# JuliaNeuralGraphics/GaussianSplatting.jl

Hardware: AMD Instinct MI355X
Metric: fwd+bwd Mpixels/s @1920x1080, 1M Gaussians SH=3 (higher is better)
Workload: dtype f32

## Files before the change

### gaussiansplatting.jl_amd/_lib.py

```python
from __future__ import annotations

import ctypes as C
import os
import subprocess

_HERE = os.path.dirname(os.path.abspath(__file__))
LIB_PATH = os.environ.get("GSR_HIP_LIB", os.path.join(_HERE, "libgsr_hip.so"))
HEADER_PATH = os.path.join(os.path.dirname(_HERE), "include", "gsr.h")

GSR_OK, GSR_E_INVALID_ARG, GSR_E_OOM, GSR_E_HIP, GSR_E_STATE = 0, -1, -2, -3, -4
DEFAULT = 0
SSIM_FAST, SSIM_EXACT = 1, 2
PREPROCESS_DIRECT, PREPROCESS_AGGREGATING = 1, 2
TUNER_OFF, TUNER_ON = 1, 2
GRAD_FP32_REFERENCE, GRAD_ACCURATE = 1, 2
MODES = {"rgb": 3, "rgbd": 5, "rgbdn": 8}
FORWARD_ONLY = 1
FLAG_REFERENCE_TILE_LISTS = 2
FLAG_ANTIALIASED = 4
ABI_VERSION = 6

(BUF_RADII, BUF_GRAD_MEANS2D, BUF_N_CONTRIB, BUF_FINAL_T, BUF_TILE_RANGES, BUF_VALUES_SORTED, BUF_GEOM, BUF_NORMALS,
 BUF_GRAD_ROWS, BUF_INSTANCE_AUX, BUF_COMPENSATIONS) = range(11)


class GsrError(RuntimeError):
    def __init__(self, code, msg):
        super().__init__(f"gsr error {code}: {msg}")
        self.code = code


class Config(C.Structure):
    _fields_ = [("width", C.c_int32), ("height", C.c_int32), ("mode", C.c_int32), ("near_plane", C.c_float),
                ("far_plane", C.c_float), ("radius_clip", C.c_int32), ("blur_eps", C.c_float), ("flags", C.c_uint32),
                ("bins_budget_bytes", C.c_uint64), ("ssim_precision", C.c_int32), ("preprocess_form", C.c_int32),
                ("form_tuner", C.c_int32), ("grad_precision", C.c_int32)]


class Inputs(C.Structure):
    _fields_ = [("n", C.c_int32), ("n_coeffs", C.c_int32), ("sh_degree", C.c_int32), ("means", C.c_void_p),
                ("shs", C.c_void_p), ("opacities", C.c_void_p), ("scales", C.c_void_p), ("rotations", C.c_void_p),
                ("background", C.c_float * 3)]


class CameraS(C.Structure):
    _fields_ = [("R", C.c_float * 9), ("t", C.c_float * 3), ("focal", C.c_float * 2), ("principal", C.c_float * 2),
                ("camera_center", C.c_float * 3), ("R_dev", C.c_void_p), ("t_dev", C.c_void_p)]


class Aux(C.Structure):
    _fields_ = [("covisibilities", C.c_void_p), ("uncertainties", C.c_void_p), ("radii", C.c_void_p),
                ("flags", C.c_uint32), ("reserved", C.c_uint32)]


class Stats(C.Structure):
    _fields_ = [("n_rendered", C.c_int64), ("n_visible", C.c_int32), ("max_tile_instances", C.c_int32),
                ("generation", C.c_uint64), ("bins_bytes", C.c_int64), ("compact_binning", C.c_int32), ("preprocess_form", C.c_int32),
                ("bins_regrowths", C.c_uint32), ("compact_fallbacks", C.c_uint32), ("tuner_rearms", C.c_uint32),
                ("scratch_regrowths", C.c_uint32), ("fused_relaunches", C.c_uint32), ("held_views", C.c_uint32),
                ("bin_capacity", C.c_uint32), ("tuner_form", C.c_int32), ("tuner_ms", C.c_float * 2),
                ("tier_tiles", C.c_uint32 * 3), ("reserved", C.c_uint32)]

    HISTORY = ("bins_regrowths", "compact_fallbacks", "tuner_rearms", "scratch_regrowths", "fused_relaunches", "held_views")

    def history(self) -> dict:
        return {k: int(getattr(self, k)) for k in self.HISTORY}


class Grads(C.Structure):
    _fields_ = [("vmeans", C.c_void_p), ("vshs", C.c_void_p), ("vopacities", C.c_void_p), ("vscales", C.c_void_p),
                ("vrotations", C.c_void_p), ("vR", C.c_void_p), ("vt", C.c_void_p), ("vcolors", C.c_void_p),
                ("vmeans2d", C.c_void_p), ("forward_generation", C.c_uint64), ("flags", C.c_uint32), ("reserved", C.c_uint32)]


GRADS_COLOR_COTANGENT = 0x1
ADAM_MAX_GROUPS = 8


class AdamGroup(C.Structure):
    _fields_ = [("theta", C.c_void_p), ("grad", C.c_void_p), ("mu", C.c_void_p), ("nu", C.c_void_p),
                ("count", C.c_int64), ("lr", C.c_float), ("current_step", C.c_uint32)]


class TailGrads(C.Structure):
    _fields_ = [("vmeans", C.c_void_p), ("vshs", C.c_void_p), ("vopacities", C.c_void_p), ("vscales", C.c_void_p),
                ("vrotations", C.c_void_p)]


class TailState(C.Structure):
    _fields_ = [("theta", C.c_void_p * 6), ("mu", C.c_void_p * 6), ("nu", C.c_void_p * 6), ("lr", C.c_float * 6),
                ("current_step", C.c_uint32 * 6), ("beta1", C.c_float), ("beta2", C.c_float), ("eps", C.c_float),
                ("scale_dims", C.c_int32), ("shs", C.c_void_p), ("opacities_act", C.c_void_p),
                ("scales_act", C.c_void_p), ("vmeans2d", C.c_void_p), ("forward_generation", C.c_uint64),
                ("flags", C.c_uint32), ("reserved", C.c_uint32)]


class ComposeGroup(C.Structure):
    _fields_ = [("src", C.c_void_p), ("dst", C.c_void_p), ("row_words", C.c_int32), ("new_zero", C.c_int32)]


class DepthAnchorS(C.Structure):
    _fields_ = [("a", C.c_float), ("b", C.c_float), ("floor", C.c_float), ("disparity", C.c_float), ("p_far", C.c_float)]


COMPOSE_MAX_GROUPS = 24
FILTER3D_CAMERA_FLOATS = 22
DENSIFY_CLONE, DENSIFY_SPLIT, DENSIFY_PRUNE = 0, 1, 2


class GatherGroup(C.Structure):
    _fields_ = [("src", C.c_void_p), ("dst", C.c_void_p), ("row_words", C.c_int32)]


class FormTuner(C.Structure):
    _fields_ = [("phase", C.c_int32), ("form", C.c_int32), ("n_ref", C.c_int32), ("age", C.c_uint32), ("ms", C.c_float * 2)]


class PolicyConfig(C.Structure):
    _fields_ = [("grid_x", C.c_int32), ("grid_y", C.c_int32), ("bins_budget_bytes", C.c_uint64), ("preprocess_form", C.c_int32),
                ("form_tuner", C.c_int32), ("beside_max_tiles", C.c_uint32), ("bwd_split_max_tiles", C.c_uint32),
                ("agg_max_bands", C.c_int32), ("reserved", C.c_int32)]


class PolicyState(C.Structure):
    _fields_ = [("bin_cap", C.c_uint32), ("compact_sticky", C.c_uint32), ("last_n", C.c_int32), ("last_max_tile", C.c_uint32),
                ("last_n_rendered", C.c_int64), ("tier_n", C.c_uint32 * 3), ("bin_cap_view", C.c_uint32), ("views", C.c_uint64),
                ("tuner", FormTuner), ("bins_regrowths", C.c_uint32), ("compact_fallbacks", C.c_uint32),
                ("compact_views", C.c_uint32), ("overflow_views", C.c_uint32), ("tuner_rearms", C.c_uint32),
                ("fused_relaunches", C.c_uint32), ("held_views", C.c_uint32), ("reserved", C.c_uint32)]


class ViewPlan(C.Structure):
    _fields_ = [("bin_cap_view", C.c_uint32), ("form_request", C.c_int32), ("form", C.c_int32), ("timed_slot", C.c_int32),
                ("skewed", C.c_int32), ("hold_fused", C.c_int32), ("tuner_decided", C.c_int32), ("spec_mid4", C.c_uint32),
                ("spec_mid8", C.c_uint32), ("reserved", C.c_int32)]


class ViewOutcome(C.Structure):
    _fields_ = [("binning", C.c_int32), ("fused_done", C.c_int32), ("long_tiles", C.c_int32), ("beside", C.c_int32),
                ("launch_fused_now", C.c_int32), ("reserved", C.c_int32), ("sorted_mid4", C.c_uint32), ("sorted_mid8", C.c_uint32),
                ("bin_cap_next", C.c_uint32), ("bins_regrown", C.c_uint32)]


class BwdSplit(C.Structure):
    _fields_ = [("n_big", C.c_uint32), ("n_mid8", C.c_uint32), ("n_mid4", C.c_uint32), ("split_len", C.c_uint32)]


POLICY_EXPORTS = ["gsr_policy_config_init", "gsr_policy_state_init", "gsr_policy_agg_plan", "gsr_policy_preprocess_form",
                  "gsr_policy_form_is_open", "gsr_policy_begin_view", "gsr_policy_end_view", "gsr_policy_bwd_split"]


def bind_policy(lib):
    P = C.POINTER
    lib.gsr_policy_config_init.argtypes = [P(PolicyConfig), C.c_int32, C.c_int32, C.c_uint64, C.c_int32]
    lib.gsr_policy_config_init.restype = None
    lib.gsr_policy_state_init.argtypes = [P(PolicyState)]
    lib.gsr_policy_state_init.restype = None
    lib.gsr_policy_agg_plan.argtypes = [C.c_int32, C.c_int32, C.c_uint32, P(C.c_int32), P(C.c_int32), P(C.c_size_t), P(C.c_int32)]
    lib.gsr_policy_agg_plan.restype = None
    lib.gsr_policy_preprocess_form.argtypes = [P(PolicyConfig), C.c_int32, C.c_int32, C.c_uint32, C.c_int32]
    lib.gsr_policy_preprocess_form.restype = C.c_int32
    lib.gsr_policy_form_is_open.argtypes = [P(PolicyConfig), C.c_int32, C.c_uint32]
    lib.gsr_policy_form_is_open.restype = C.c_int32
    lib.gsr_policy_begin_view.argtypes = [P(PolicyConfig), P(PolicyState), C.c_int32, P(C.c_float), P(ViewPlan)]
    lib.gsr_policy_begin_view.restype = None
    lib.gsr_policy_end_view.argtypes = [P(PolicyConfig), P(PolicyState), P(ViewPlan), C.c_int64, C.c_uint32, C.c_uint32, C.c_uint32,
                                        C.c_uint32, C.c_uint64, C.c_int32, P(ViewOutcome)]
    lib.gsr_policy_end_view.restype = None
    lib.gsr_policy_bwd_split.argtypes = [P(PolicyConfig), C.c_uint32, C.c_uint32, C.c_uint32, P(BwdSplit)]
    lib.gsr_policy_bwd_split.restype = None
    lib.gsr_bins_capacity_after.argtypes = [C.c_int64, C.c_int32, C.c_int32, C.c_int32, C.c_uint64, C.c_uint32]
    lib.gsr_bins_capacity_after.restype = C.c_uint32
    return lib


EXPORTS = ["gsr_create", "gsr_destroy", "gsr_release_scene_buffers", "gsr_memory_usage", "gsr_debug_check_guards", "gsr_reserve", "gsr_drop_forward", "gsr_bins_capacity_after", "gsr_forward",
           "gsr_backward", "gsr_host_wait_policy", "gsr_buffer", "gsr_copy_buffer", "gsr_ssim_forward", "gsr_ssim_backward", "gsr_loss_l1_ssim",
           "gsr_ssim_precision", "gsr_get_ssim_precision", "gsr_preprocess_form", "gsr_get_preprocess_form",
           "gsr_allreduce_grads", "gsr_last_error_string", "gsr_version", "gsr_abi_version", "gsr_check_abi", "gsr_profile_enable",
           "gsr_profile_stage_count", "gsr_profile_stages", "gsr_profile_stage_name", "gsr_profile_read", "gsr_profile_read_intervals", "gsr_update_stats",
           "gsr_prologue_forward", "gsr_prologue_backward", "gsr_adam_step", "gsr_stream_triad",
           "gsr_mask_findall_scratch_bytes", "gsr_mask_findall", "gsr_gather_rows", "gsr_sh_grad_from_views", "gsr_sh_grad_from_views_tail", "gsr_trainer_tail_step",
           "gsr_backward_trainer_tail",
           "gsr_densify_grad_mean", "gsr_densify_mask", "gsr_compose_rows", "gsr_split_transform", "gsr_reset_opacity", "gsr_morton_codes",
           "gsr_knn_scratch_bytes", "gsr_knn_scales",
           "gsr_filter3d_scratch_bytes", "gsr_filter3d_compute", "gsr_filter3d_apply", "gsr_filter3d_apply_backward",
           "gsr_tsdf_integrate", "gsr_mesh_scratch_bytes", "gsr_mesh_count", "gsr_mesh_emit",
           "gsr_ply_pack_rows", "gsr_ply_unpack_rows", "gsr_count_nonfinite",
           "gsr_bilateral_scratch_bytes", "gsr_bilateral_tv_scratch_bytes", "gsr_bilateral_slice_forward",
           "gsr_bilateral_slice_backward", "gsr_bilateral_tv", "gsr_bilateral_adam_tail",
           "gsr_normal_loss_scratch_bytes", "gsr_normal_loss_forward", "gsr_normal_loss_backward",
           "gsr_flatten_loss_scratch_bytes", "gsr_flatten_loss",
           "gsr_depth_loss_scratch_bytes", "gsr_depth_target", "gsr_depth_loss_forward", "gsr_depth_loss_backward",
           "gsr_sky_scratch_bytes", "gsr_sky_composite_forward", "gsr_sky_composite_backward",
           "gsr_eval_scratch_bytes", "gsr_eval_metrics", "gsr_frame_rgb8",
           "gsr_frames_scratch_bytes", "gsr_depth_scale", "gsr_frame_depth16", "gsr_frame_normal8", "gsr_pick_point",
           "gsr_mcmc_weights", "gsr_mcmc_sample_scratch_bytes", "gsr_mcmc_sample", "gsr_mcmc_split_sampled",
           "gsr_mcmc_relocation_params", "gsr_mcmc_relocate_rows", "gsr_mcmc_inject_noise",
           "gsr_mcmc_regularization_scratch_bytes", "gsr_mcmc_regularization"] + POLICY_EXPORTS

_lib = None


def build(verbose: bool = False) -> str:
    cmd = ["make", "-C", os.path.join(_HERE, "csrc"), "-j4"]
    r = subprocess.run(cmd, capture_output=True, text=True)
    if verbose or r.returncode != 0:
        print(r.stdout[-4000:], r.stderr[-4000:])
    if r.returncode != 0:
        raise RuntimeError("building libgsr_hip.so failed")
    return LIB_PATH


def build_tools(verbose: bool = False) -> bool:
    r = subprocess.run(["make", "-C", os.path.join(_HERE, "csrc"), "tools"], capture_output=True, text=True)
    if verbose or r.returncode != 0:
        print(r.stdout[-2000:], r.stderr[-2000:])
    return r.returncode == 0


def load():
    global _lib
    if _lib is not None:
        return _lib
    if not os.path.exists(LIB_PATH):
        raise RuntimeError(f"{LIB_PATH} is missing: run __graft_entry__.build() (there is no CPU fallback)")
    import torch
    lib = C.CDLL(LIB_PATH)
    vp, i32, f32 = C.c_void_p, C.c_int, C.c_float
    lib.gsr_create.argtypes = [C.POINTER(Config), C.POINTER(vp)]
    lib.gsr_destroy.argtypes = [vp]
    lib.gsr_release_scene_buffers.argtypes = [vp]
    lib.gsr_memory_usage.argtypes = [vp]
    lib.gsr_memory_usage.restype = C.c_int64
    lib.gsr_debug_check_guards.argtypes = [vp]
    lib.gsr_reserve.argtypes = [vp, C.c_int64, C.c_int64]
    lib.gsr_drop_forward.argtypes = [vp]
    bind_policy(lib)
    lib.gsr_forward.argtypes = [vp, C.POINTER(Inputs), C.POINTER(CameraS), vp, C.POINTER(Aux), vp, C.POINTER(Stats)]
    lib.gsr_backward.argtypes = [vp, C.POINTER(Inputs), C.POINTER(CameraS), vp, C.POINTER(Grads), vp]
    lib.gsr_host_wait_policy.argtypes = [i32, i32, i32]
    lib.gsr_buffer.argtypes = [vp, i32, C.POINTER(vp), C.POINTER(C.c_size_t)]
    lib.gsr_copy_buffer.argtypes = [vp, i32, vp, C.c_size_t, vp]
    lib.gsr_ssim_forward.argtypes = [i32, i32, i32, i32, vp, vp, f32, f32, i32, vp, vp, vp, vp, vp]
    lib.gsr_ssim_backward.argtypes = [i32, i32, i32, i32, vp, vp, vp, vp, vp, vp, vp, vp]
    lib.gsr_loss_l1_ssim.argtypes = [vp, vp, vp, f32, vp, vp, vp]
    lib.gsr_allreduce_grads.argtypes = [vp, vp, C.c_size_t, vp]
    lib.gsr_update_stats.argtypes = [vp, vp, vp, vp, vp]
    lib.gsr_prologue_forward.argtypes = [i32, i32, i32, vp, vp, vp, vp, vp, vp, vp, vp]
    lib.gsr_prologue_backward.argtypes = [i32, i32, i32, vp, vp, vp, vp, vp, vp, vp, vp, vp, vp]
    lib.gsr_adam_step.argtypes = [C.POINTER(AdamGroup), i32, f32, f32, f32, vp]
    lib.gsr_mask_findall_scratch_bytes.argtypes = [C.c_int64]
    lib.gsr_mask_findall_scratch_bytes.restype = C.c_size_t
    lib.gsr_mask_findall.argtypes = [vp, C.c_int64, vp, vp, vp, vp]
    lib.gsr_gather_rows.argtypes = [C.POINTER(GatherGroup), i32, vp, C.c_int64, vp]
    i64 = C.c_int64
    lib.gsr_densify_grad_mean.argtypes = [i64, vp, vp, vp, vp]
    lib.gsr_densify_mask.argtypes = [C.c_int32, i64, i64, vp, vp, C.c_int32, vp, vp, f32, f32, f32, C.c_int32, vp, vp]
    lib.gsr_compose_rows.argtypes = [C.POINTER(ComposeGroup), C.c_int32, vp, i64, vp, i64, C.c_int32, vp]
    lib.gsr_split_transform.argtypes = [i64, C.c_int32, vp, vp, vp, C.c_uint32, vp]
    lib.gsr_reset_opacity.argtypes = [i64, vp, vp]
    lib.gsr_morton_codes.argtypes = [i64, vp, C.POINTER(C.c_float), C.POINTER(C.c_float), vp, vp]
    lib.gsr_knn_scratch_bytes.argtypes = [i64]
    lib.gsr_knn_scratch_bytes.restype = C.c_size_t
    lib.gsr_knn_scales.argtypes = [i64, vp, vp, f32, C.c_int32, vp, vp, vp, C.c_size_t, vp]
    lib.gsr_filter3d_scratch_bytes.argtypes = [i64]
    lib.gsr_filter3d_scratch_bytes.restype = C.c_size_t
    lib.gsr_filter3d_compute.argtypes = [i64, vp, C.c_int32, vp, f32, f32, vp, vp, vp, vp, C.c_size_t, vp]
    lib.gsr_filter3d_apply.argtypes = [i64, vp, vp, vp, C.c_int32, vp, vp, vp]
    lib.gsr_filter3d_apply_backward.argtypes = [i64, vp, vp, vp, vp, vp, vp, vp, vp]
    lib.gsr_tsdf_integrate.argtypes = [C.c_int32, C.c_int32, C.c_int32, vp, f32, f32, C.c_int32, C.c_int32, C.c_int32, vp,
                                       C.POINTER(CameraS), f32, f32, vp, vp, vp]
    lib.gsr_mesh_scratch_bytes.argtypes = [C.c_int32, C.c_int32, C.c_int32]
    lib.gsr_mesh_scratch_bytes.restype = C.c_size_t
    lib.gsr_mesh_count.argtypes = [C.c_int32, C.c_int32, C.c_int32, vp, vp, vp, C.c_size_t, vp]
    lib.gsr_mesh_emit.argtypes = [C.c_int32, C.c_int32, C.c_int32, vp, f32, vp, vp, vp, C.c_size_t, i64, i64, vp, vp, vp, vp]
    lib.gsr_count_nonfinite.argtypes = [C.POINTER(vp), C.POINTER(C.c_int32), C.c_int32, i64, vp, vp, vp]
    lib.gsr_ply_pack_rows.argtypes = [i64, C.c_int32, vp, vp, vp, vp, vp, vp, vp, vp]
    lib.gsr_ply_unpack_rows.argtypes = [i64, C.c_int32, vp, vp, vp, vp, vp, vp, vp, vp]
    lib.gsr_sh_grad_from_views.argtypes = [i32, i32, i32, i32, vp, vp, vp, vp, vp]
    lib.gsr_sh_grad_from_views_tail.argtypes = [i32, i32, i32, i32, vp, vp, C.POINTER(TailGrads), C.POINTER(TailState), vp]
    lib.gsr_trainer_tail_step.argtypes = [i32, i32, i32, C.POINTER(TailGrads), C.POINTER(vp), C.POINTER(vp), C.POINTER(vp),
                                          C.POINTER(f32), C.POINTER(C.c_uint32), f32, f32, f32, vp, vp, vp, vp]
    lib.gsr_backward_trainer_tail.argtypes = [vp, C.POINTER(Inputs), C.POINTER(CameraS), vp, C.POINTER(TailState), vp]
    sz = C.c_size_t
    lib.gsr_bilateral_scratch_bytes.argtypes = [i32] * 5
    lib.gsr_bilateral_scratch_bytes.restype = sz
    lib.gsr_bilateral_tv_scratch_bytes.argtypes = [i32]
    lib.gsr_bilateral_tv_scratch_bytes.restype = sz
    lib.gsr_bilateral_slice_forward.argtypes = [i32, i32, i32, vp, vp, i32, i32, i32, vp, vp]
    lib.gsr_bilateral_slice_backward.argtypes = [i32, i32, i32, vp, vp, i32, i32, i32, vp, vp, vp, vp, sz, vp]
    lib.gsr_bilateral_tv.argtypes = [i32, i32, i32, i32, vp, f32, vp, vp, vp, sz, vp]
    lib.gsr_bilateral_adam_tail.argtypes = [i32, i32, i32, i32, vp, vp, vp, vp, i32, f32, f32, C.c_uint32, f32, f32, f32,
                                            vp, vp, sz, vp]
    lib.gsr_normal_loss_scratch_bytes.argtypes = [i32, i32]
    lib.gsr_normal_loss_scratch_bytes.restype = sz
    lib.gsr_normal_loss_forward.argtypes = [i32, i32, i32, vp, C.POINTER(CameraS), f32, vp, vp, vp, vp, sz, vp]
    lib.gsr_normal_loss_backward.argtypes = [i32, i32, i32, vp, C.POINTER(CameraS), f32, vp, vp, sz, vp]
    lib.gsr_flatten_loss_scratch_bytes.argtypes = [i32]
    lib.gsr_flatten_loss_scratch_bytes.restype = sz
    lib.gsr_flatten_loss.argtypes = [i32, i32, vp, f32, vp, vp, vp, sz, vp]
    lib.gsr_depth_loss_scratch_bytes.argtypes = [i32, i32]
    lib.gsr_depth_loss_scratch_bytes.restype = sz
    lib.gsr_depth_target.argtypes = [i32, i32, vp, C.POINTER(DepthAnchorS), f32, vp, vp, vp, vp]
    lib.gsr_depth_loss_forward.argtypes = [i32, i32, i32, vp, vp, C.POINTER(DepthAnchorS), f32, f32, f32, vp, vp, vp, vp, vp,
                                           vp, sz, vp]
    lib.gsr_depth_loss_backward.argtypes = [i32, i32, i32, vp, vp, C.POINTER(DepthAnchorS), f32, f32, f32, vp, vp, sz, vp]
    lib.gsr_sky_scratch_bytes.argtypes = [i32, i32]
    lib.gsr_sky_scratch_bytes.restype = sz
    lib.gsr_sky_composite_forward.argtypes = [i32, i32, i32, vp, vp, vp, f32, vp, vp, vp, vp]
    lib.gsr_sky_composite_backward.argtypes = [i32, i32, i32, vp, vp, vp, f32, vp, vp, vp, vp]
    lib.gsr_eval_scratch_bytes.argtypes = [i32, i32]
    lib.gsr_eval_scratch_bytes.restype = sz
    lib.gsr_eval_metrics.argtypes = [i32, i32, i32, vp, vp, vp, vp, i32, vp, vp, vp, vp]
    lib.gsr_frame_rgb8.argtypes = [i32, i32, i32, vp, vp, i32, vp, vp]
    lib.gsr_frames_scratch_bytes.argtypes = [i32, i32]
    lib.gsr_frames_scratch_bytes.restype = sz
    lib.gsr_depth_scale.argtypes = [i32, i32, i32, vp, f32, C.c_double, vp, vp, vp]
    lib.gsr_frame_depth16.argtypes = [i32, i32, i32, vp, i32, f32, f32, vp, i32, vp, vp]
    lib.gsr_frame_normal8.argtypes = [i32, i32, i32, vp, f32, C.POINTER(C.c_float * 9), vp, vp]
    lib.gsr_pick_point.argtypes = [i32, i32, i32, vp, C.POINTER(CameraS), i32, i32, i32, vp, vp]
    u32 = C.c_uint32
    lib.gsr_mcmc_weights.argtypes = [i64, i32, vp, vp, f32, f32, vp, vp, vp]
# ... 44 lines not shown
```

### gaussiansplatting.jl_amd/csrc/composite.hip

```cpp
#include "gsr_kernels.h"
#include "gsr_dispatch.h"
#include "wave_reduce.h"
#include "tile_sort_device.h"


namespace {

struct Bg { float v[8]; };

__device__ __forceinline__ unsigned long long wave_ballot(bool p) { return __builtin_amdgcn_ballot_w64(p); }

struct SigmaX { float hxx, bdx; };
__device__ __forceinline__ SigmaX sigma_x(float ha, float b, float dx) {
    return SigmaX{__fmul_rn(ha, __fmul_rn(dx, dx)), __fmul_rn(b, dx)};
}
__device__ __forceinline__ float sigma_of(const SigmaX sx, float hc, float dy, float dy2) {
    return __fmaf_rn(sx.bdx, dy, __fmaf_rn(hc, dy2, sx.hxx));
}
__device__ __forceinline__ float alpha_of(float opacity, float G) { return fminf(0.99f, __fmul_rn(opacity, G)); }

template <int C, int N> struct LdsSplats {
    float4 q[C > 3 ? 4 : 3][N];
    __device__ __forceinline__ const float4& operator()(int plane, int j) const { return q[plane][j]; }
    __device__ __forceinline__ float4& operator()(int plane, int j) { return q[plane][j]; }
// ... 131 lines not shown
template <int C, bool AUX>
__global__ __launch_bounds__(64) void composite_fwd_strip_kernel(int W, int H, int grid_x,
                                                                 const uint32_t* __restrict__ tile_start,
                                                                 const uint32_t* __restrict__ tile_order,
                                                                 GsrStream stream, Bg bg, float* __restrict__ image,
                                                                 uint32_t* __restrict__ n_contrib,
                                                                 float* __restrict__ final_T,
                                                                 const uint32_t* __restrict__ values_sorted,
                                                                 uint8_t* __restrict__ covis,
                                                                 float* __restrict__ uncert, GsrTierLists tiers) {
    __shared__ LdsSplats<C, 64> e;
    const int id = blockIdx.x, k = id >> 3;
    const int quad = k & 3;
    const int slot = ((k >> 2) << 3) | (id & 7);
    int tile;
    if (tile_order) {
        if (slot >= grid_x * ((H + GSR_TILE - 1) / GSR_TILE)) return;
        tile = (int)tile_order[slot];
    } else {
        if ((uint32_t)slot >= tiers.n_big + tiers.n_mid8 + tiers.n_mid4) return;
        GSR_TIER_TILE(tile, tiers, (uint32_t)slot);
        if (tiers.split_len) __builtin_amdgcn_s_setprio(3);
    }
    composite_fwd_quadrant<C, AUX>(W, H, grid_x, tile, quad, (int)threadIdx.x, tile_start, stream, bg, image,
                                   n_contrib, final_T, values_sorted, covis, uncert, e);
}

template <int C, bool AUX, bool KEEP>
__global__ __launch_bounds__(256) __attribute__((amdgpu_waves_per_eu(8))) void sort_composite_fwd_kernel(int W, int H, int grid_x,
                                                                 const uint32_t* __restrict__ tile_start,
                                                                 const uint32_t* __restrict__ tile_order,
                                                                 uint32_t* __restrict__ tile_count,
                                                                 const uint64_t* __restrict__ bins, uint32_t bin_cap,
                                                                 GsrGeom geom, GsrStream stream, Bg bg,
                                                                 float* __restrict__ image,
                                                                 uint32_t* __restrict__ n_contrib,
                                                                 float* __restrict__ final_T,
                                                                 uint32_t* __restrict__ values_sorted,
                                                                 uint32_t* __restrict__ ranges,
                                                                 uint8_t* __restrict__ covis, float* __restrict__ uncert,
                                                                 const uint32_t* __restrict__ totals,
                                                                 uint32_t cap_instances) {
    constexpr int CHUNK = 256;
    __shared__ uint32_t ids[1024];
    __shared__ LdsSplats<C, CHUNK> e;
    if (totals[GSR_TOTAL_D] > cap_instances || (totals[GSR_TOTAL_MAX_LIST] > bin_cap && bin_cap < 1024u)) return;
    const int tile = (int)tile_order[blockIdx.x];
    const int tid = threadIdx.x, lane = tid & 63, wave = tid >> 6;
    const uint32_t start = tile_start[tile], end = tile_start[tile + 1];
    const uint32_t n = end - start;
    if (tid == 0) {
        tile_count[tile] = 0u;
        ranges[2 * tile] = n ? start : 0u;
        ranges[2 * tile + 1] = n ? end : 0u;
    }
    if (n > 1024u) return;
    const int tile_x = tile % grid_x, tile_y = tile / grid_x;
    const int X0 = tile_x * GSR_TILE, Y0 = tile_y * GSR_TILE;
    const int quad = wave;
    const uint32_t strip_bits = 0x10000u << quad;
    const int px = X0 + 8 * (quad & 1) + (lane & 7), py = Y0 + 8 * (quad >> 1) + (lane >> 3);
    const bool inside = px < W && py < H;
    float fx = (float)px, fy = (float)py;
    asm volatile("" : "+v"(fx), "+v"(fy));
    FwdPixel<C> p;
    fwd_pixel_init<C>(p, inside);
    if (n > 0) {
        if (wave == (int)(blockIdx.x & 3u)) gsr_sort::wave_sort_ids_any(ids, n, lane, bins + (size_t)tile * bin_cap);
        __syncthreads();
        for (uint32_t cbase = 0; cbase < n; cbase += CHUNK) {
            const uint32_t i = cbase + (uint32_t)tid;
            if (i < n) {
                const uint32_t id = ids[i];
                const gsr_sort::InstanceVals v = gsr_sort::instance_vals<C>(id, X0, Y0, geom);
                if (KEEP) {
                    const uint32_t pos = start + i;
                    values_sorted[pos] = id;
                    stream.s0[pos] = v.v0; stream.s1[pos] = v.v1; stream.s2[pos] = v.v2;
                    if (C > 3) stream.s3[pos] = v.v3;
                }
                e(0, tid) = v.v0; e(1, tid) = v.v1;
                e(2, tid) = make_float4(v.v2.x, __uint_as_float(i + 1u), v.v2.z, v.v2.w);
                if (C > 3) e(C > 3 ? 3 : 0, tid) = v.v3;
            }
            __syncthreads();
            const int cnt = (int)min((uint32_t)CHUNK, n - cbase);
            for (int b = 0; b < cnt; b += 64) {
                if (p.done == ~0ull) break;
                const int k = b + lane;
                const bool cand = k < cnt && (__float_as_uint(e(2, k).w) & strip_bits) != 0u;
                const unsigned long long m = wave_ballot(cand);
                if (m == 0ull) continue;
                fwd_blend_selected<C, AUX, CHUNK>(p, m, e, b, fx, fy, ids + cbase + b, covis);
            }
            if (cbase + CHUNK < n) __syncthreads();
        }
    }
    fwd_pixel_store<C, AUX>(p, inside, px, py, W, bg, image, n_contrib, final_T, uncert);
}

template <int C> struct AccRow { static constexpr int N = C == 3 ? 9 : (C == 5 ? 10 : 13); static constexpr int STRIDE = N | 1; };

template <bool ACC> __device__ __forceinline__ float bwd_exp_neg(float sigma) { return ACC ? expf(-sigma) : __expf(-sigma); }
template <bool ACC> __device__ __forceinline__ float bwd_rcp(float x) { return ACC ? __fdiv_rn(1.0f, x) : __builtin_amdgcn_rcpf(x); }


template <int C, int VC>
__device__ __forceinline__ void bwd_store_row(float4* rows, const float4 a, const float4 b, float slot,
                                              const float (&r)[AccRow<VC>::N]) {
    constexpr int NA = AccRow<VC>::N;
    const float mo = -b.y, mh = -0.5f * b.y;
    float4* row = rows + (size_t)GSR_ROW_F4(C) * __float_as_uint(slot);
    row[0] = make_float4(r[0], r[1], r[2], r[3]);
    row[1] = make_float4(mh * r[4], mh * r[5], mh * r[6], VC > 3 ? r[9 < NA ? 9 : 0] : 0.0f);
    row[2] = make_float4(mo * (2.0f * a.z * r[7] + a.w * r[8]), mo * (a.w * r[7] + 2.0f * b.x * r[8]),
                         VC > 5 ? r[10 < NA ? 10 : 0] : 0.0f, VC > 5 ? r[11 < NA ? 11 : 0] : 0.0f);
    if (C > 5) row[3] = make_float4(VC > 5 ? r[12 < NA ? 12 : 0] : 0.0f, 0.0f, 0.0f, 0.0f);
}

template <int C>
__device__ __forceinline__ void bwd_zero_rows(float4* rows, const GsrStream stream, uint32_t p, uint32_t end) {
    for (; p < end; p += 64) {
        float4* row = rows + (size_t)GSR_ROW_F4(C) * __float_as_uint(stream.s2[p].y);
        const float4 z = make_float4(0.0f, 0.0f, 0.0f, 0.0f);
        row[0] = z; row[1] = z; row[2] = z;
        if (C > 5) row[3] = z;
    }
}

template <int C>
__device__ __forceinline__ uint32_t bwd_stage_entry(const GsrStream& stream, uint32_t p, int k, float4* l0, float4* l1,
                                                    float4* l2, float4* l3) {
    l0[k] = stream.s0[p];
    l1[k] = stream.s1[p];
    const float4 t2 = stream.s2[p];
    l2[k] = make_float4(t2.x, t2.w, t2.z, t2.y);
    if (C > 3) l3[k] = stream.s3[p];
    return __float_as_uint(t2.w);
}


template <int C, bool BG0, int VC = C, bool ACC = false>
__global__ __launch_bounds__(64, 1) void composite_bwd_kernel(int W, int H, int grid_x,
                                                 const uint32_t* __restrict__ tile_start,
                                                 const uint32_t* __restrict__ tile_order,
                                                 GsrStream stream, Bg bg,
                                                 const float* __restrict__ vpixels,
                                                 const uint32_t* __restrict__ n_contrib,
                                                 const float* __restrict__ final_T, GsrInst inst,
                                                 GsrTierLists tiers) {
    static_assert(!(C == 3 && BG0), ":rgb on a zero background is composite_bwd_kernel_rgb_bg0");
#include "composite_bwd_body.inc"
}
__global__ __attribute__((amdgpu_flat_work_group_size(1, 64), amdgpu_waves_per_eu(6, 6)))
void composite_bwd_kernel_rgb_bg0(int W, int H, int grid_x,
                                                 const uint32_t* __restrict__ tile_start,
                                                 const uint32_t* __restrict__ tile_order,
                                                 GsrStream stream, Bg bg,
                                                 const float* __restrict__ vpixels,
                                                 const uint32_t* __restrict__ n_contrib,
                                                 const float* __restrict__ final_T, GsrInst inst,
                                                 GsrTierLists tiers) {
    constexpr int C = 3, VC = 3;
    constexpr bool BG0 = true, ACC = false;
#include "composite_bwd_body.inc"
}

constexpr int LONG_SEGS = GSR_BWD_LONG_SEGS;

template <int C, bool BG0, int PASS>
__global__ __launch_bounds__(64) void composite_bwd_long_kernel(int W, int H, int grid_x,
                                                                const uint32_t* __restrict__ tile_start,
                                                                GsrStream stream, Bg bg,
                                                                const float* __restrict__ vpixels,
                                                                const uint32_t* __restrict__ n_contrib,
                                                                const float* __restrict__ final_T, GsrInst inst,
                                                                GsrTierLists tiers, float2* __restrict__ state) {
    constexpr int VC = C, BB = 64, ROWS = 16, wave = 0;
    constexpr bool ACC = false, FY_REBUILD = false;
    constexpr int NA = AccRow<C>::N, ST = AccRow<C>::STRIDE, PPL = 4;
    __shared__ float4 l0[BB], l1[BB], l2[BB];
    __shared__ float4 l3[C > 3 ? BB : 1];
    __shared__ float my[BB * ST];
    __builtin_amdgcn_s_setprio(3);
    const int lane = threadIdx.x;
    const uint32_t listed = blockIdx.x / LONG_SEGS;
    const int g = (int)(blockIdx.x % LONG_SEGS);
    const gsr::LaneBits lane_bits(lane);
    const int red_slot = gsr::wave_reduce_index<NA>(lane);
    const bool red_writer = gsr::wave_reduce_writer(lane);
    const gsr::RowColConsts rowcol(lane);
    const gsr::RowColConstsD rowcol_d(lane);
    int tile;
    GSR_TIER_TILE(tile, tiers, listed);
    const int tile_x = tile % grid_x, tile_y = tile / grid_x;
    const int px = tile_x * GSR_TILE + (lane & 15);
    const int py0 = tile_y * GSR_TILE + (lane >> 4);
    const float fx = (float)px;
    const uint32_t start = tile_start[tile], end = tile_start[tile + 1];
    if (end == start) return;
    float fy[PPL], T[PPL], A[PPL], bgT[BG0 ? 1 : PPL], vp[PPL][C];
    int last_contributor[PPL];
#include "composite_bwd_state.inc"
    int tile_last = deepest;
#pragma unroll
    for (int off = 32; off > 0; off >>= 1) tile_last = max(tile_last, __shfl_xor(tile_last, off));
    tile_last = __builtin_amdgcn_readfirstlane(tile_last);
    const int seg = (((tile_last + LONG_SEGS - 1) / LONG_SEGS) + 63) & ~63;
    const int hi = tile_last - g * seg, lo = max(0, hi - seg);
    float2* const st_tile = state + (size_t)listed * LONG_SEGS * 256;
    if (PASS == 2 && g == 0) bwd_zero_rows<C>(inst.rows, stream, start + (uint32_t)tile_last + lane, end);
    if (hi <= 0) {
        if (PASS == 1) {
#pragma unroll
            for (int q = 0; q < PPL; q++) st_tile[(size_t)g * 256 + lane + 64 * q] = make_float2(1.0f, 0.0f);
        }
        return;
    }

    auto stage = [&](int top , int cnt) -> unsigned long long {
        __builtin_amdgcn_wave_barrier();
        uint32_t mask = 0u;
        if (lane < cnt) mask = bwd_stage_entry<C>(stream, start + (uint32_t)(top - 1 - lane), lane, l0, l1, l2, l3);
        __builtin_amdgcn_fence(__ATOMIC_RELEASE, "wavefront");
        __builtin_amdgcn_wave_barrier();
        return wave_ballot(lane < cnt && (mask & 0xFFFFu) != 0u);
    };

    if (PASS == 1) {
        float m_[PPL], c_[PPL];
#pragma unroll
        for (int q = 0; q < PPL; q++) { m_[q] = 1.0f; c_[q] = 0.0f; }
        for (int top = hi; top > lo; top -= 64) {
            const int cnt = min(64, top - lo);
            unsigned long long wl = stage(top, cnt);
            while (wl) {
                const int j = __builtin_ctzll(wl);
                wl &= wl - 1;
                const int contributor = top - 1 - j;
#include "composite_bwd_decode.inc"
#pragma unroll
                for (int q = 0; q < PPL; q++) {
                    if (__builtin_amdgcn_readfirstlane((int)((entry_rowbits >> (4 * q)) & 0xFu)) == 0) continue;
                    const float dy = a.y - fy[q], dy2 = __fmul_rn(dy, dy);
                    const float sigma = sigma_of(sx, b.x, dy, dy2);
                    if (contributor < last_contributor[q] && __float_as_uint(sigma) < thr_bits) {
                        const float alpha = alpha_of(o, __expf(-sigma));
                        float cv = f[0] * vp[q][0];
#pragma unroll
                        for (int c = 1; c < C; c++) cv += f[c] * vp[q][c];
                        c_[q] = c_[q] + alpha * (cv - c_[q]);
                        m_[q] = m_[q] * (1.0f - alpha);
                    }
                }
            }
        }
#pragma unroll
        for (int q = 0; q < PPL; q++) st_tile[(size_t)g * 256 + lane + 64 * q] = make_float2(m_[q], c_[q]);
        return;
    }

    for (int k = 0; k < g; k++) {
#pragma unroll
        for (int q = 0; q < PPL; q++) {
            const float2 mc = st_tile[(size_t)k * 256 + lane + 64 * q];
            T[q] = T[q] / mc.x;
            A[q] = mc.x * A[q] + mc.y;
        }
    }
    for (int top = hi; top > lo; top -= 64) {
        const int cnt = min(64, top - lo);
        unsigned long long wl = stage(top, cnt);
        unsigned long long touched[1] = {0ull};
        while (wl) {
            const int j = __builtin_ctzll(wl);
            wl &= wl - 1;
            const int contributor = top - 1 - j;
#include "composite_bwd_visit.inc"
#include "composite_bwd_reduce.inc"
        }
        __builtin_amdgcn_fence(__ATOMIC_ACQ_REL, "wavefront");
        __builtin_amdgcn_wave_barrier();
        if (lane < cnt) {
            float r[NA];
            const bool hit = (touched[0] >> lane) & 1ull;
#pragma unroll
            for (int k = 0; k < NA; k++) r[k] = hit ? my[lane * ST + k] : 0.0f;
            bwd_store_row<C, C>(inst.rows, l0[lane], l1[lane], l2[lane].w, r);
        }
    }
}

bool bg_is_zero(const Bg& b) {
    for (int c = 0; c < 8; c++)
        if (b.v[c] != 0.0f) return false;
    return true;
}

Bg make_bg(const float* background, int channels) {
    Bg b;
    for (int c = 0; c < 8; c++) b.v[c] = (c < 3 && c < channels) ? background[c] : 0.0f;
    return b;
}

}

void gsr_launch_composite_fwd(hipStream_t s, int channels, GsrCam cam, GsrTiles tiles, GsrStream stream, GsrFrame frame,
                              const GsrTierLists* only_listed) {
    const uint32_t* const tile_order = only_listed ? nullptr : tiles.order;
    const GsrTierLists tiers = only_listed ? *only_listed : GsrTierLists{};
    const int n_slots = tile_order ? cam.grid_x * cam.grid_y : (int)(tiers.n_big + tiers.n_mid8 + tiers.n_mid4);
    if (n_slots <= 0) return;
    dim3 grid(32 * ((n_slots + 7) / 8)), block(64);
    Bg bg = make_bg(frame.background, channels);
    gsr::dispatch_channels(channels, [&](auto c) {
        constexpr int CH = c;
        gsr::dispatch_bool(frame.covis || frame.uncert, [&](auto a) {
            constexpr bool AUX = a;
            hipLaunchKernelGGL((composite_fwd_strip_kernel<CH, AUX>), grid, block, 0, s, cam.width, cam.height, cam.grid_x,
                               tiles.start, tile_order, stream, bg, frame.image, frame.n_contrib, frame.final_T,
                               frame.values_sorted, frame.covis, frame.uncert, tiers);
        });
    });
}

void gsr_launch_sort_composite_fwd(hipStream_t s, int channels, GsrCam cam, GsrTiles tiles, GsrKeys keys, GsrGeom geom,
                                   GsrStream stream, GsrFrame frame, uint32_t cap_instances, bool keep_backward_state) {
    dim3 grid(cam.grid_x * cam.grid_y), block(256);
    Bg bg = make_bg(frame.background, channels);
    gsr::dispatch_channels(channels, [&](auto c) {
        constexpr int CH = c;
        gsr::dispatch_bool(frame.covis || frame.uncert, [&](auto a) {
            constexpr bool AUX = a;
            gsr::dispatch_bool(keep_backward_state, [&](auto k) {
                constexpr bool KEEP = k;
                hipLaunchKernelGGL((sort_composite_fwd_kernel<CH, AUX, KEEP>), grid, block, 0, s, cam.width, cam.height,
                                   cam.grid_x, tiles.start, tiles.order, tiles.count, keys.bins, keys.cap, geom, stream, bg,
                                   frame.image, frame.n_contrib, frame.final_T, frame.values_sorted, tiles.ranges,
                                   frame.covis, frame.uncert, tiles.totals, cap_instances);
            });
        });
    });
}

void gsr_launch_composite_bwd(hipStream_t s, int channels, GsrCam cam, GsrTiles tiles, GsrStream stream, GsrFrame frame,
                              const float* vpixels, GsrInst inst, uint32_t split_len, bool color_only, bool accurate) {
    dim3 grid(cam.grid_x * cam.grid_y), block(64);
    Bg bg = make_bg(frame.background, channels);
    GsrTierLists none{};
    none.split_len = split_len;
    const bool bg0 = bg_is_zero(bg);
#define LAUNCH_K(CC, ZZ, VV, AA)                                                                                       \
    hipLaunchKernelGGL((composite_bwd_kernel<CC, ZZ, VV, AA>), grid, block, 0, s, cam.width, cam.height,               \
                       cam.grid_x, tiles.start, tiles.order, stream, bg, vpixels, frame.n_contrib, frame.final_T, inst, none)
#define LAUNCH2(CC, ZZ) do { if (accurate) LAUNCH_K(CC, false, CC, true); else LAUNCH_K(CC, ZZ, CC, false); } while (0)
#define LAUNCH3(CC, ZZ) do { if (accurate) LAUNCH_K(CC, false, 3, true); else LAUNCH_K(CC, ZZ, 3, false); } while (0)
    if (channels == 3) {
        if (bg0 && !accurate)
            hipLaunchKernelGGL(composite_bwd_kernel_rgb_bg0, grid, block, 0, s, cam.width, cam.height, cam.grid_x, tiles.start, tiles.order,
                               stream, bg, vpixels, frame.n_contrib, frame.final_T, inst, none);
        else LAUNCH2(3, false);
    }
    else if (color_only) {
        if (channels == 5) LAUNCH3(5, false); else LAUNCH3(8, false);
    }
    else if (channels == 5) { if (bg0) LAUNCH2(5, true); else LAUNCH2(5, false); }
    else if (bg0) LAUNCH2(8, true);
    else LAUNCH2(8, false);
#undef LAUNCH_K
#undef LAUNCH2
#undef LAUNCH3
}

void gsr_launch_composite_bwd_listed(hipStream_t s, int channels, GsrCam cam, GsrTiles tiles, GsrTierLists tiers,
                                     GsrStream stream, GsrFrame frame, const float* vpixels, GsrInst inst, float* long_state) {
    const uint32_t n_listed = tiers.n_big + tiers.n_mid8 + tiers.n_mid4;
    if (n_listed == 0) return;
    Bg bg = make_bg(frame.background, channels);
    dim3 grid(n_listed * LONG_SEGS), block(64);
    float2* st = reinterpret_cast<float2*>(long_state);
    gsr::dispatch_channels(channels, [&](auto c) {
        constexpr int CH = c;
        gsr::dispatch_bool(bg_is_zero(bg), [&](auto z) {
            constexpr bool BG0 = z;
            hipLaunchKernelGGL((composite_bwd_long_kernel<CH, BG0, 1>), grid, block, 0, s, cam.width, cam.height, cam.grid_x,
                               tiles.start, stream, bg, vpixels, frame.n_contrib, frame.final_T, inst, tiers, st);
            hipLaunchKernelGGL((composite_bwd_long_kernel<CH, BG0, 2>), grid, block, 0, s, cam.width, cam.height, cam.grid_x,
                               tiles.start, stream, bg, vpixels, frame.n_contrib, frame.final_T, inst, tiers, st);
        });
    });
}
```

### gaussiansplatting.jl_amd/csrc/gsr_api.cpp

```cpp
#include <algorithm>
#include <atomic>
#include <cstdlib>
#include <new>

#include "gsr_kernels.h"
#include "adam_math.h"
#include "gsr_host.h"
#include "gsr_devbuf.h"
#include "gsr_profiler.h"
#include "gsr_host_wait.h"
#include "gsr_sizes.h"

using namespace gsr_host;

thread_local char gsr_host::g_err[512] = "";

namespace {

struct TunerEvents {
    hipEvent_t ev[2 * GSR_TUNER_TIMED_VIEWS] = {};
    bool create() {
        for (auto& e : ev)
            if (!e && hipEventCreate(&e) != hipSuccess) { e = nullptr; return false; }
        return true;
    }
    void destroy() { for (auto& e : ev) if (e) { (void)hipEventDestroy(e); e = nullptr; } }
    bool read(float ms[GSR_TUNER_TIMED_VIEWS]) {
        for (int v = 0; v < GSR_TUNER_TIMED_VIEWS; v++) {
            const hipError_t q = hipEventQuery(ev[2 * v + 1]);
            if (q == hipErrorNotReady) { (void)hipGetLastError(); return false; }
            if (q != hipSuccess || hipEventElapsedTime(&ms[v], ev[2 * v], ev[2 * v + 1]) != hipSuccess) return false;
        }
        return true;
    }
};

constexpr int kHandleBufs = 33;

bool valid_mode(int m) { return m == GSR_MODE_RGB || m == GSR_MODE_RGBD || m == GSR_MODE_RGBDN; }

}

struct gsr_handle {
    gsr_config cfg;
    int grid_x, grid_y, n_tiles;
    DevBuf ranges, n_contrib, final_T, tile_count, tile_start, tile_order, totals;
    DevBuf geo, gnormal, radii, bsum, bpre, bvis;
    DevBuf comp;
    gsr_policy_config pcfg;
    gsr_policy_state pol;
    TunerEvents tuner_ev;
    int last_form = 0;
    bool last_compact = false;
    bool tile_count_dirty = false;
    double wait_ema_us = 0.0;
    DevBuf bins, keys_compact, big_list, values_sorted, s0, s1, s2, s3, big_scratch, long_state;
    DevBuf overflow_fill;
    DevBuf rows, vmean2d;
    DevBuf pose_part;
    DevBuf d0, d1, d2, partial;
    uint32_t* host_totals = nullptr;
    uint32_t* host_totals_dev = nullptr;
    uint32_t totals_seq = 0;
    hipStream_t aux_stream = nullptr;
    hipEvent_t ev_fork = nullptr, ev_join = nullptr;
    bool fwd_valid = false, bwd_valid = false;
    bool fwd_only = false;
    bool inputs_consumed = false;
    bool dropped_by_reserve = false;
    uint64_t generation = 0;
    int32_t* radii_cur = nullptr;
    float2* vmean2d_cur = nullptr;
    int last_n = 0;
    int64_t last_D = 0;
    int64_t last_slots = 0;
    const float* loss_vpixels = nullptr;
    uint64_t loss_generation = 0;
    uint32_t reserved_regrowths = 0;
    DevBuf dbg_flag;
    Profiler prof;

    DevBuf* all[kHandleBufs];
    int n_all = 0;
    GuardDamage guard_damage;
};

std::atomic<int> gsr_host::g_ssim_exact{[] { const char* e = getenv("GSR_SSIM_EXACT"); return e && e[0] == '1' ? 1 : 0; }()};

namespace {

struct BufRow {
    DevBuf gsr_handle::*buf;
    const char* name;
    bool scene, fill_ok;
    uint32_t guard_word;
};
#define BUF(member, scene, fill_ok, guard_word) {&gsr_handle::member, #member, scene, fill_ok, guard_word}
constexpr BufRow kBufs[] = {
    BUF(ranges, false, false, 1u),
    BUF(n_contrib, false, false, 1u),
    BUF(final_T, false, true, 1u),
    BUF(tile_count, false, false, 1u),
    BUF(tile_start, false, false, 1u),
    BUF(tile_order, false, false, 0u),
    BUF(totals, false, false, 1u),
    BUF(geo, true, false, 1u),
    BUF(gnormal, true, true, 1u),
    BUF(radii, true, false, 1u),
    BUF(bsum, true, false, 1u),
    BUF(bpre, true, false, 1u),
    BUF(bvis, true, false, 1u),
    BUF(bins, true, false, 1u),
    BUF(values_sorted, true, false, 0u),
    BUF(s0, true, false, 1u),
    BUF(s1, true, false, 1u),
    BUF(s2, true, false, 1u),
    BUF(s3, true, false, 1u),
    BUF(big_scratch, true, false, 1u),
    BUF(rows, true, true, 1u),
    BUF(vmean2d, true, true, 1u),
    BUF(d0, false, true, 1u),
    BUF(d1, false, true, 1u),
    BUF(d2, false, true, 1u),
    BUF(partial, false, true, 1u),
    BUF(keys_compact, true, false, 1u),
    BUF(big_list, false, false, 0u),
    BUF(long_state, false, true, 1u),
    BUF(overflow_fill, false, false, 1u),
    BUF(dbg_flag, false, false, 1u),
    BUF(pose_part, true, true, 1u),
    BUF(comp, true, true, 1u),
};
#undef BUF
template <class Pred> constexpr int count_bufs(Pred pred) {
    int n = 0;
    for (const BufRow& r : kBufs) n += pred(r) ? 1 : 0;
    return n;
}
static_assert(sizeof(kBufs) / sizeof(kBufs[0]) == kHandleBufs, "gsr_handle::all holds one pointer per row");
static_assert(count_bufs([](const BufRow& r) { return r.scene; }) == 18, "the scene buffers");
static_assert(count_bufs([](const BufRow& r) { return r.fill_ok; }) == 11, "the GSR_DEBUG_FILL candidates");
static_assert(count_bufs([](const BufRow& r) { return r.guard_word == 0u; }) == 3, "the id buffers whose guard word is 0");

bool antialiased(const gsr_handle* h) { return (h->cfg.flags & GSR_FLAG_ANTIALIASED) != 0u; }

GsrCam make_cam(const gsr_handle* h, const gsr_camera* c) {
    GsrCam k;
    for (int r = 0; r < 3; r++)
        for (int col = 0; col < 3; col++) k.R[r * 3 + col] = c->R[col * 3 + r];
    for (int i = 0; i < 3; i++) { k.t[i] = c->t[i]; k.center[i] = c->camera_center[i]; }
    for (int i = 0; i < 2; i++) { k.focal[i] = c->focal[i]; k.principal[i] = c->principal[i]; }
    k.width = h->cfg.width; k.height = h->cfg.height;
    k.grid_x = h->grid_x; k.grid_y = h->grid_y;
    k.near_plane = h->cfg.near_plane; k.far_plane = h->cfg.far_plane;
    k.radius_clip = h->cfg.radius_clip; k.blur_eps = h->cfg.blur_eps;
    k.exact_cull = (h->cfg.flags & GSR_FLAG_REFERENCE_TILE_LISTS) ? 0 : 1;
    k.R_dev = c->R_dev; k.t_dev = c->t_dev;
    return k;
}

float* comp_of(const gsr_handle* h) { return antialiased(h) ? h->comp.as<float>() : nullptr; }
GsrGeom geom_of(const gsr_handle* h) {
    return GsrGeom{h->geo.as<GsrGeoRec>(), h->gnormal.as<float4>(), h->radii_cur, h->bsum.as<uint32_t>(),
                   h->bpre.as<uint32_t>()};
}
GsrStream stream_of(const gsr_handle* h) {
    return GsrStream{h->s0.as<float4>(), h->s1.as<float4>(), h->s2.as<float4>(), h->s3.as<float4>()};
}
GsrInst inst_of(const gsr_handle* h) { return GsrInst{h->rows.as<float4>()}; }
GsrTiles tiles_of(const gsr_handle* h) {
    return GsrTiles{h->tile_start.as<uint32_t>(), h->tile_count.as<uint32_t>(), h->tile_order.as<uint32_t>(),
                    h->ranges.as<uint32_t>(), h->big_list.as<uint32_t>(), h->totals.as<uint32_t>(), h->n_tiles, h->grid_x};
}
GsrKeys bins_of(const gsr_handle* h, uint32_t cap) { return GsrKeys{h->bins.as<uint64_t>(), cap, nullptr}; }
GsrFrame frame_of(const gsr_handle* h, const float* background, float* image, const gsr_aux* aux) {
    return GsrFrame{background, image, h->n_contrib.as<uint32_t>(), h->final_T.as<float>(), h->values_sorted.as<uint32_t>(),
                    aux ? aux->covisibilities : nullptr, aux ? aux->uncertainties : nullptr};
}

std::atomic<int> g_preprocess_form{[] { const char* e = getenv("GSR_PREPROCESS_AGG"); return e ? (atoi(e) != 0 ? 1 : 0) : -1; }()};
inline int ssim_exact_of(const gsr_handle* h) {
    return h->cfg.ssim_precision != GSR_DEFAULT ? (h->cfg.ssim_precision == GSR_SSIM_EXACT ? 1 : 0)
                                                : g_ssim_exact.load(std::memory_order_relaxed);
}
inline int preprocess_form_of(const gsr_handle* h) {
    return h->cfg.preprocess_form != GSR_DEFAULT ? (h->cfg.preprocess_form == GSR_PREPROCESS_AGGREGATING ? 1 : 0)
                                                 : g_preprocess_form.load(std::memory_order_relaxed);
}

gsr_gaussian_bytes gaussian_bytes(const gsr_handle* h, int64_t n) {
    return gsr_sizes_per_gaussian((size_t)n, h->cfg.mode, gsr_pose_partial_floats(n), antialiased(h));
}

void fill_history(const gsr_handle* h, gsr_stats* st) {
    const gsr_policy_state& p = h->pol;
    st->bins_regrowths = p.bins_regrowths;
    st->compact_fallbacks = p.compact_fallbacks;
    st->tuner_rearms = p.tuner_rearms;
    uint32_t grows = 0;
    for (int i = 0; i < h->n_all; i++) grows += h->all[i]->regrowths;
    st->scratch_regrowths = grows - h->reserved_regrowths;
    st->fused_relaunches = p.fused_relaunches;
    st->held_views = p.held_views;
    const bool decided = p.tuner.phase == GSR_TUNER_TIMED_VIEWS + 1;
    st->tuner_form = decided ? p.tuner.form : -1;
    st->tuner_ms[0] = decided ? p.tuner.ms[0] : 0.0f;
    st->tuner_ms[1] = decided ? p.tuner.ms[1] : 0.0f;
}

__global__ void nonzero_tail_kernel(const float* __restrict__ v, size_t n_pixels, int C, uint32_t* flag) {
    const size_t p = (size_t)blockIdx.x * blockDim.x + threadIdx.x;
    if (p >= n_pixels) return;
    bool bad = false;
    for (int c = 3; c < C; c++) bad |= v[p * C + c] != 0.0f;
    if (bad) atomicOr(flag, 1u);
}
int check_color_cotangent(gsr_handle* h, const float* vpixels, hipStream_t s) {
    if (h->cfg.mode <= 3) return GSR_OK;
    if (vpixels != h->loss_vpixels || h->loss_generation != h->generation)
        return fail(GSR_E_INVALID_ARG, "GSR_GRADS_COLOR_COTANGENT is only valid for the cotangent gsr_loss_l1_ssim wrote for this "
                    "forward on this handle (its vpixels %p for forward #%llu; got %p for forward #%llu): a cotangent with depth / "
                    "alpha / normal terms must not set the flag", (const void*)h->loss_vpixels,
                    (unsigned long long)h->loss_generation, (const void*)vpixels, (unsigned long long)h->generation);
    const char* look = getenv("GSR_CHECK_COLOR_COTANGENT");
    if (!(look && look[0] == '1')) return GSR_OK;
    int rc = h->dbg_flag.ensure(4);
    if (rc) return rc;
    const size_t P = (size_t)h->cfg.width * h->cfg.height;
    uint32_t bad = 0;
    HIPCHK(hipMemsetAsync(h->dbg_flag.p, 0, 4, s));
    hipLaunchKernelGGL(nonzero_tail_kernel, dim3((unsigned)((P + 255) / 256)), dim3(256), 0, s, vpixels, P, h->cfg.mode,
                       h->dbg_flag.as<uint32_t>());
    HIPCHK(hipMemcpyAsync(&bad, h->dbg_flag.p, 4, hipMemcpyDeviceToHost, s));
    HIPCHK(hipStreamSynchronize(s));
    if (bad) return fail(GSR_E_INVALID_ARG, "GSR_GRADS_COLOR_COTANGENT: vpixels holds non-zero values above the colour channels "
                         "(something was added to the loss head's cotangent in place)");
    return GSR_OK;
}

int check_inputs(const gsr_handle* h, const gsr_inputs* in, const gsr_camera* cam) {
    if (!h || !in || !cam) return fail(GSR_E_INVALID_ARG, "null handle / inputs / camera");
    if (in->n < 0) return fail(GSR_E_INVALID_ARG, "n = %d < 0", in->n);
    if (in->sh_degree < 0 || in->sh_degree > 3) return fail(GSR_E_INVALID_ARG, "sh_degree = %d not in 0..3", in->sh_degree);
    if (in->n_coeffs < (in->sh_degree + 1) * (in->sh_degree + 1) || in->n_coeffs > 16)
        return fail(GSR_E_INVALID_ARG, "n_coeffs = %d does not hold degree %d", in->n_coeffs, in->sh_degree);
    if (in->n > 0 && (!in->means || !in->shs || !in->opacities || !in->scales || !in->rotations))
        return fail(GSR_E_INVALID_ARG, "null input array");
    if (((uintptr_t)in->rotations & 15) != 0) return fail(GSR_E_INVALID_ARG, "rotations must be 16-byte aligned");
    if ((cam->R_dev == nullptr) != (cam->t_dev == nullptr))
        return fail(GSR_E_INVALID_ARG, "R_dev and t_dev must be given together");
    return GSR_OK;
}

}

extern "C" {

const char* gsr_last_error_string(void) { return g_err; }
#define GSR_STR2(x) #x
#define GSR_STR(x) GSR_STR2(x)
const char* gsr_version(void) { return "gsr-hip 0.4 abi " GSR_STR(GSR_ABI_VERSION) " (gfx950)"; }
int gsr_abi_version(void) { return GSR_ABI_VERSION; }

int gsr_host_wait_policy(int spin_us, int yield_us, int sleep_us) {
    if (spin_us < 0 || yield_us < 0 || sleep_us < 0) return fail(GSR_E_INVALID_ARG, "negative wait time");
    if (spin_us > kWaitMaxUs || yield_us > kWaitMaxUs || sleep_us > kWaitMaxUs)
        return fail(GSR_E_INVALID_ARG, "wait times are at most %d us", kWaitMaxUs);
    WaitPolicy w;
    w.spin_us = spin_us; w.yield_us = yield_us; w.sleep_us = sleep_us;
    g_wait_packed.store(pack_wait(w), std::memory_order_relaxed);
    return GSR_OK;
}

int gsr_ssim_precision(int exact) {
    if (exact != 0 && exact != 1) return fail(GSR_E_INVALID_ARG, "gsr_ssim_precision: 0 (fast) or 1 (exact)");
    g_ssim_exact.store(exact, std::memory_order_relaxed);
    return GSR_OK;
}
int gsr_get_ssim_precision(void) { return g_ssim_exact.load(std::memory_order_relaxed); }

int gsr_preprocess_form(int form) {
    if (form < -1 || form > 1) return fail(GSR_E_INVALID_ARG, "gsr_preprocess_form: -1 (by size), 0 (direct) or 1 (aggregating)");
    g_preprocess_form.store(form, std::memory_order_relaxed);
    return GSR_OK;
}
int gsr_get_preprocess_form(void) { return g_preprocess_form.load(std::memory_order_relaxed); }

int gsr_check_abi(int abi_version, size_t sizeof_config, size_t sizeof_inputs, size_t sizeof_camera, size_t sizeof_aux,
                  size_t sizeof_stats, size_t sizeof_grads, size_t sizeof_tail_state) {
    if (abi_version != GSR_ABI_VERSION)
        return fail(GSR_E_INVALID_ARG, "binding was written for gsr ABI %d, this library is ABI %d", abi_version, GSR_ABI_VERSION);
    const struct { const char* name; size_t theirs, ours; } t[] = {
        {"gsr_config", sizeof_config, sizeof(gsr_config)}, {"gsr_inputs", sizeof_inputs, sizeof(gsr_inputs)},
        {"gsr_camera", sizeof_camera, sizeof(gsr_camera)}, {"gsr_aux", sizeof_aux, sizeof(gsr_aux)},
// ... 256 lines not shown
    sc1.close();
    v.seq = ++h->totals_seq ? h->totals_seq : ++h->totals_seq;
    StageScope sc2(h->prof, ST_SCAN, s);
    gsr_launch_tile_scan(s, tiles_of(h), geom_of(h), (v.n + 255) / 256, h->bvis.as<uint32_t>(), h->host_totals_dev, v.seq);
    sc2.close();
    HIPCHK(hipGetLastError());
    uint64_t cap_instances = std::min(std::min(h->values_sorted.cap / 4, h->s0.cap / 16), std::min(h->s1.cap / 16, h->s2.cap / 16));
    if (v.C > 3) cap_instances = std::min<uint64_t>(cap_instances, h->s3.cap / 16);
    cap_instances = std::min<uint64_t>(cap_instances, 0xFFFFFFFFull);
    if (v.fwd_only) cap_instances = 0xFFFFFFFFull;
    v.cap_instances = cap_instances;
    v.spec = use_bins && cap_instances > 0;
    const bool hold_fused = v.spec && v.plan.hold_fused;
    if (v.spec && !hold_fused) launch_fused(h, v, s);
    if (!(hold_fused && !v.fwd_only)) v.plan.spec_mid4 = v.plan.spec_mid8 = 0u;
    if (v.plan.spec_mid4 | v.plan.spec_mid8) {
        StageScope scs(h->prof, ST_SORT, s, true);
        gsr_launch_tile_sort_mid(s, v.C, tiles_of(h), bins_of(h, bin_cap_view), v.plan.spec_mid4, v.plan.spec_mid8, geom_of(h),
                                 stream_of(h), h->values_sorted.as<uint32_t>(), (uint32_t)cap_instances);
        scs.close();
    }
    return GSR_OK;
}

static void fill_view_stats(const gsr_handle* h, const FwdView& v, gsr_stats* st) {
    const bool hybrid = v.oc.binning == GSR_BINNING_OVERFLOW, compact = v.oc.binning == GSR_BINNING_COMPACT;
    st->n_rendered = (int64_t)v.D;
    st->n_visible = (int32_t)(v.visible & 0x7FFFFFFFu);
    st->max_tile_instances = (int32_t)v.max_tile;
    st->compact_binning = v.oc.binning;
    st->preprocess_form = h->last_form;
    st->bins_bytes = (int64_t)(compact ? v.D * 8 : (uint64_t)(h->n_tiles + 1) * v.plan.bin_cap_view * 8ull + (hybrid ? v.D * 8 : 0));
    st->bin_capacity = v.plan.bin_cap_view;
    st->tier_tiles[0] = v.n_mid4; st->tier_tiles[1] = v.n_mid8; st->tier_tiles[2] = v.n_big;
    st->reserved = 0;
    fill_history(h, st);
}

static int fwd_read_back(gsr_handle* h, FwdView& v) {
    int rc;
    if ((rc = wait_totals(h->host_totals + GSR_TOTAL_SEQ, &h->wait_ema_us, v.seq, v.s))) return rc;
    const uint32_t* t = h->host_totals;
    v.D = t[GSR_TOTAL_D]; v.D_slots = t[GSR_TOTAL_SLOTS]; v.max_tile = t[GSR_TOTAL_MAX_LIST];
    v.n_big = t[GSR_TOTAL_BIG]; v.n_mid4 = t[GSR_TOTAL_MID4]; v.n_mid8 = t[GSR_TOTAL_MID8]; v.visible = t[GSR_TOTAL_VISIBLE];
    gsr_policy_end_view(&h->pcfg, &h->pol, &v.plan, (int64_t)v.D, v.max_tile, v.n_mid4, v.n_mid8, v.n_big, v.cap_instances,
                        v.spec ? 1 : 0, &v.oc);
    h->last_n = v.n;
    h->last_D = (int64_t)v.D;
    h->last_slots = (int64_t)v.D_slots;
    h->last_compact = v.oc.binning == GSR_BINNING_COMPACT;
    if (v.stats) fill_view_stats(h, v, v.stats);
    return GSR_OK;
}

static int fwd_empty_view(gsr_handle* h, const FwdView& v) {
    const hipStream_t s = v.s;
    const size_t P = (size_t)h->cfg.width * h->cfg.height, T = (size_t)h->n_tiles;
    h->tile_count_dirty = false;
    if (v.k.exact_cull && (v.visible >> 31)) {
        gsr_launch_fill_background(s, P, v.C, frame_of(h, v.in->background, v.image_out, v.aux));
    } else {
        HIPCHK(hipMemsetAsync(v.image_out, 0, P * v.C * 4, s));
        HIPCHK(hipMemsetAsync(h->n_contrib.p, 0, P * 4, s));
        HIPCHK(hipMemsetAsync(h->final_T.p, 0, P * 4, s));
    }
    HIPCHK(hipMemsetAsync(h->ranges.p, 0, 2 * T * 4, s));
    if (v.aux && v.aux->uncertainties) HIPCHK(hipMemsetAsync(v.aux->uncertainties, 0, P * 4, s));
    h->fwd_valid = true;
    return GSR_OK;
}

static int fwd_instance_buffers(gsr_handle* h, FwdView& v) {
    int rc;
    const gsr_instance_bytes b = gsr_sizes_per_instance(v.D, v.D_slots, v.C);
    const float slack = 1.25f;
    const bool need_stream = !(v.fwd_only && v.oc.fused_done && !v.oc.long_tiles);
    if (need_stream &&
        ((rc = h->values_sorted.ensure(b.values_sorted, slack)) ||
         (rc = h->s0.ensure(b.stream, slack)) || (rc = h->s1.ensure(b.stream, slack)) ||
         (rc = h->s2.ensure(b.stream, slack)) || (v.C > 3 && (rc = h->s3.ensure(b.s3, slack)))))
        return rc;
    if (!v.fwd_only && (rc = h->rows.ensure(b.rows, slack))) return rc;
    v.slab_stride = 0;
    if (v.n_big > 0) {
        v.slab_stride = ((size_t)v.max_tile + 63) & ~(size_t)63;
        if ((rc = h->big_scratch.ensure((size_t)v.n_big * 2 * v.slab_stride * 8 + (size_t)(2 * v.n_big + 2) * 4 + 64))) return rc;
    }
    return GSR_OK;
}

static int fwd_sort_and_walk(gsr_handle* h, const FwdView& v) {
    int rc;
    const hipStream_t s = v.s;
    const size_t T = (size_t)h->n_tiles;
    const float slack = 1.25f;
    const bool fused_done = v.oc.fused_done != 0, beside = v.oc.beside != 0;
    if (v.oc.launch_fused_now) launch_fused(h, v, s);
    if (fused_done && !v.oc.long_tiles) return GSR_OK;
    StageScope sc4(h->prof, ST_SORT, s);
    GsrKeys keys = bins_of(h, v.plan.bin_cap_view);
    if (v.oc.binning == GSR_BINNING_COMPACT) {
        if ((rc = h->keys_compact.ensure(v.D * 8, slack))) return rc;
        HIPCHK(hipMemsetAsync(h->tile_count.p, 0, (T + 2) * 4, s));
        gsr_launch_emit_compact(s, v.n, v.k, geom_of(h), h->tile_start.as<uint32_t>(), h->tile_count.as<uint32_t>(),
                                h->keys_compact.as<uint64_t>(), v.max_tile, 0u);
        keys = GsrKeys{h->keys_compact.as<uint64_t>(), 0u, nullptr};
    } else if (v.oc.binning == GSR_BINNING_OVERFLOW) {
        if ((rc = h->keys_compact.ensure(v.D * 8, slack)) || (rc = h->overflow_fill.ensure((T + 2) * 4))) return rc;
        HIPCHK(hipMemsetAsync(h->overflow_fill.p, 0, (T + 2) * 4, s));
        gsr_launch_emit_compact(s, v.n, v.k, geom_of(h), h->tile_start.as<uint32_t>(), h->overflow_fill.as<uint32_t>(),
                                h->keys_compact.as<uint64_t>(), v.max_tile, keys.cap);
        keys.overflow = h->keys_compact.as<uint64_t>();
    }
    gsr_launch_tile_sort(s, v.C, !fused_done, tiles_of(h), keys, v.n_mid4, v.n_mid8, v.n_big, v.oc.sorted_mid4,
                         v.oc.sorted_mid8, h->big_scratch.as<uint64_t>(), v.slab_stride, geom_of(h), stream_of(h),
                         h->values_sorted.as<uint32_t>());
    sc4.close();
    const hipStream_t ws = beside ? h->aux_stream : s;
    if (beside) {
        HIPCHK(hipEventRecord(h->ev_fork, s));
        HIPCHK(hipStreamWaitEvent(h->aux_stream, h->ev_fork, 0));
    }
    StageScope sc5(h->prof, ST_COMPOSITE_FWD, ws);
    const GsrTierLists tiers{h->big_list.as<uint32_t>(), (uint32_t)h->n_tiles, v.n_big, v.n_mid8, v.n_mid4, beside ? 1u : 0u};
    gsr_launch_composite_fwd(ws, v.C, v.k, tiles_of(h), stream_of(h), frame_of(h, v.in->background, v.image_out, v.aux),
                             fused_done ? &tiers : nullptr);
    sc5.close();
    if (beside) {
        HIPCHK(hipEventRecord(h->ev_join, h->aux_stream));
        launch_fused(h, v, s);
        HIPCHK(hipStreamWaitEvent(s, h->ev_join, 0));
    }
    return GSR_OK;
}

int gsr_forward(gsr_handle* h, const gsr_inputs* in, const gsr_camera* cam, float* image_out, const gsr_aux* aux,
                void* stream_v, gsr_stats* stats) {
    FwdView v;
    int rc;
    if ((rc = fwd_begin(h, in, cam, image_out, aux, stream_v, stats, v))) return rc;
    if ((rc = fwd_plan_and_bin(h, v))) return rc;
    if ((rc = fwd_read_back(h, v))) return rc;
    if (v.D == 0) return fwd_empty_view(h, v);
    if ((rc = fwd_instance_buffers(h, v))) return rc;
    if ((rc = fwd_sort_and_walk(h, v))) return rc;
    h->tile_count_dirty = false;
    HIPCHK(hipGetLastError());
    if (stats) fill_history(h, stats);
    h->fwd_valid = true;
    return GSR_OK;
}

static int launch_composite_bwd(gsr_handle* h, hipStream_t s, int C, const GsrCam& k, const float* background,
                                const float* vpixels, bool color_only) {
    color_only = color_only && C > 3;
    gsr_bwd_split sp;
    gsr_policy_bwd_split(&h->pcfg, h->pol.tier_n[0], h->pol.tier_n[1], h->pol.tier_n[2], &sp);
    const bool accurate = h->cfg.grad_precision != GSR_DEFAULT;
    if (accurate) { sp.n_big = sp.n_mid8 = sp.n_mid4 = 0; sp.split_len = 0xFFFFFFFFu; }
    GsrTierLists tiers{h->big_list.as<uint32_t>(), (uint32_t)h->n_tiles, sp.n_big, sp.n_mid8, sp.n_mid4, sp.split_len};
    const uint32_t n = sp.n_big + sp.n_mid8 + sp.n_mid4;
    const GsrFrame frame = frame_of(h, background, nullptr, nullptr);
    if (n > 0) {
        int rc = h->long_state.ensure((size_t)n * GSR_BWD_LONG_SEGS * 256 * 2 * sizeof(float));
        if (rc) return rc;
        HIPCHK(hipEventRecord(h->ev_fork, s));
        HIPCHK(hipStreamWaitEvent(h->aux_stream, h->ev_fork, 0));
        gsr_launch_composite_bwd_listed(h->aux_stream, C, k, tiles_of(h), tiers, stream_of(h), frame, vpixels, inst_of(h),
                                        h->long_state.as<float>());
        HIPCHK(hipEventRecord(h->ev_join, h->aux_stream));
    }
    gsr_launch_composite_bwd(s, C, k, tiles_of(h), stream_of(h), frame, vpixels, inst_of(h), tiers.split_len, color_only, accurate);
    if (n > 0) HIPCHK(hipStreamWaitEvent(s, h->ev_join, 0));
    return GSR_OK;
}

static int check_backward_state(const gsr_handle* h, const gsr_inputs* in, const char* entry) {
    if (!h->fwd_valid && h->dropped_by_reserve)
        return fail(GSR_E_STATE, "%s: a gsr_reserve that reallocated scratch (or gsr_drop_forward) dropped the handle's last "
                    "forward; run gsr_forward again", entry);
    if (!h->fwd_valid || h->last_n != in->n)
        return fail(GSR_E_STATE, "%s without a matching gsr_forward on this handle", entry);
    if (h->fwd_only)
        return fail(GSR_E_STATE, "the handle's last forward was GSR_FORWARD_ONLY: it kept no backward state");
    if (h->inputs_consumed)
        return fail(GSR_E_STATE, "the inputs of the handle's last forward were updated in place by "
                    "gsr_backward_trainer_tail; run gsr_forward again");
    return GSR_OK;
}

static int composite_bwd_stage(gsr_handle* h, hipStream_t s, const gsr_inputs* in, const gsr_camera* cam, const float* vpixels,
                               float* vmeans2d, uint32_t flags, GsrCam* k) {
    int rc;
    if (!vmeans2d && (rc = h->vmean2d.ensure(gaussian_bytes(h, in->n).vmean2d, 1.25f))) return rc;
    h->vmean2d_cur = vmeans2d ? reinterpret_cast<float2*>(vmeans2d) : h->vmean2d.as<float2>();
    const bool color_only = (flags & GSR_GRADS_COLOR_COTANGENT) != 0u;
    if (color_only && (rc = check_color_cotangent(h, vpixels, s))) return rc;
    *k = make_cam(h, cam);
    StageScope sc(h->prof, ST_COMPOSITE_BWD, s);
    if (h->last_D > 0 && (rc = launch_composite_bwd(h, s, h->cfg.mode, *k, in->background, vpixels, color_only))) return rc;
    sc.close();
    return GSR_OK;
}

int gsr_backward(gsr_handle* h, const gsr_inputs* in, const gsr_camera* cam, const float* vpixels,
                 const gsr_grads* g, void* stream_v) {
    int rc = check_inputs(h, in, cam);
    if (rc) return rc;
    if (!vpixels || !g) return fail(GSR_E_INVALID_ARG, "null vpixels / grads");
    if ((rc = check_backward_state(h, in, "gsr_backward"))) return rc;
    if ((g->flags & ~GSR_GRADS_COLOR_COTANGENT) != 0u || g->reserved != 0u) return fail(GSR_E_INVALID_ARG, "unknown gsr_grads.flags / reserved bits");
    if (g->forward_generation != 0 && g->forward_generation != h->generation)
        return fail(GSR_E_STATE, "gsr_backward for forward #%llu, but the handle's last forward is #%llu (another "
                    "gsr_forward ran in between)", (unsigned long long)g->forward_generation,
                    (unsigned long long)h->generation);
    if (in->n > 0 && (!g->vmeans || (!g->vshs && !g->vcolors) || !g->vopacities || !g->vscales || !g->vrotations))
        return fail(GSR_E_INVALID_ARG, "null gradient buffer");
    if ((g->vR == nullptr) != (g->vt == nullptr)) return fail(GSR_E_INVALID_ARG, "vR and vt must be given together");
    if (((uintptr_t)g->vrotations & 15) != 0) return fail(GSR_E_INVALID_ARG, "vrotations must be 16-byte aligned");
    hipStream_t s = (hipStream_t)stream_v;
    const int C = h->cfg.mode, n = in->n;
    if (n == 0) return GSR_OK;
    if (g->vR && (rc = h->pose_part.ensure(gaussian_bytes(h, n).pose_part, 1.25f))) return rc;
    GsrCam k;
    if ((rc = composite_bwd_stage(h, s, in, cam, vpixels, g->vmeans2d, g->flags, &k))) return rc;
    StageScope sc8(h->prof, ST_PERGAUSS_BWD, s);
    gsr_launch_pergauss_bwd(s, n, in->n_coeffs, in->sh_degree, C, in->means, in->scales, in->rotations, in->shs, k,
                            geom_of(h), inst_of(h), h->vmean2d_cur, g->vmeans, g->vshs, g->vopacities,
                            g->vscales, g->vrotations, g->vR, g->vt, h->pose_part.as<float>(), g->vcolors,
                            h->cfg.grad_precision == GSR_GRAD_FP32_REFERENCE,
                            antialiased(h) ? in->opacities : nullptr, comp_of(h));
    sc8.close();
    HIPCHK(hipGetLastError());
    h->bwd_valid = true;
    return GSR_OK;
}

static int buffer_lookup(const gsr_handle* h, int which, const void** dev_ptr, size_t* bytes) {
    const size_t n = (size_t)h->last_n, P = (size_t)h->cfg.width * h->cfg.height, T = (size_t)h->n_tiles;
    const gsr_gaussian_bytes gb = n ? gaussian_bytes(h, h->last_n) : gsr_gaussian_bytes{};
    const gsr_instance_bytes ib = gsr_sizes_per_instance((uint64_t)h->last_D, (uint64_t)h->last_slots, h->cfg.mode);
    const DevBuf* b = nullptr;
    size_t sz = 0;
    switch (which) {
        case GSR_BUF_RADII:
            *dev_ptr = h->fwd_valid && n ? h->radii_cur : nullptr;
            *bytes = *dev_ptr ? gb.radii : 0;
            return GSR_OK;
        case GSR_BUF_GRAD_MEANS2D:
            *dev_ptr = h->bwd_valid && n ? h->vmean2d_cur : nullptr;
            *bytes = *dev_ptr ? gb.vmean2d : 0;
            return GSR_OK;
        case GSR_BUF_COMPENSATIONS:
            *dev_ptr = h->fwd_valid && n && gb.comp && gb.comp <= h->comp.cap ? h->comp.p : nullptr;
            *bytes = *dev_ptr ? gb.comp : 0;
            return GSR_OK;
        case GSR_BUF_N_CONTRIB: b = &h->n_contrib; sz = P * 4; break;
        case GSR_BUF_FINAL_T: b = &h->final_T; sz = P * 4; break;
        case GSR_BUF_TILE_RANGES: b = &h->ranges; sz = 2 * T * 4; break;
        case GSR_BUF_VALUES_SORTED: b = &h->values_sorted; sz = h->fwd_only ? 0 : ib.values_sorted; break;
        case GSR_BUF_GEOM: b = &h->geo; sz = gb.geo; break;
        case GSR_BUF_NORMALS: b = &h->gnormal; sz = gb.gnormal; break;
        case GSR_BUF_GRAD_ROWS: b = &h->rows; sz = (size_t)h->last_slots * 16 * GSR_ROW_F4(h->cfg.mode); break;
        case GSR_BUF_INSTANCE_AUX: b = &h->s2; sz = h->fwd_only ? 0 : ib.stream; break;
        default: return fail(GSR_E_INVALID_ARG, "unknown buffer id %d", which);
    }
    if (sz > b->cap) sz = 0;
    *dev_ptr = sz ? b->p : nullptr;
    *bytes = sz;
    return GSR_OK;
}

int gsr_buffer(const gsr_handle* h, int which, const void** dev_ptr, size_t* bytes) {
    if (!h || !dev_ptr || !bytes) return fail(GSR_E_INVALID_ARG, "null argument");
    return buffer_lookup(h, which, dev_ptr, bytes);
}

int gsr_copy_buffer(const gsr_handle* h, int which, void* dst, size_t bytes, void* stream) {
    if (!h || (!dst && bytes)) return fail(GSR_E_INVALID_ARG, "null argument");
    const void* src = nullptr;
    size_t have = 0;
    int rc = buffer_lookup(h, which, &src, &have);
    if (rc) return rc;
    if (bytes > have) return fail(GSR_E_STATE, "buffer %d holds %zu bytes, %zu requested (not produced yet?)", which, have, bytes);
    if (bytes) HIPCHK(hipMemcpyAsync(dst, src, bytes, hipMemcpyDeviceToDevice, (hipStream_t)stream));
    return GSR_OK;
}

int gsr_loss_l1_ssim(gsr_handle* h, const float* image, const float* target, float lambda_dssim, float* loss_out,
                     float* vpixels, void* stream) {
    if (!h || !image || !target || !loss_out || !vpixels) return fail(GSR_E_INVALID_ARG, "null argument");
    hipStream_t s = (hipStream_t)stream;
    const int W = h->cfg.width, H = h->cfg.height, C = h->cfg.mode;
    const size_t P = (size_t)W * H;
    if (P * C > 0xFFFFFFFFull) return fail(GSR_E_INVALID_ARG, "image too large for the loss head");
    const int exact = ssim_exact_of(h);
    int rc;
    if ((rc = h->d0.ensure(3 * P * 4)) || (rc = h->d1.ensure(3 * P * 4)) || (rc = h->d2.ensure(3 * P * 4)) ||
        (rc = h->partial.ensure((exact ? gsr_loss_partial_pairs_exact : gsr_loss_partial_pairs_fast)(W, H) * 2 * 4)))
        return rc;
    const float C1 = 0.01f * 0.01f, C2 = 0.03f * 0.03f;
    StageScope sc9(h->prof, ST_LOSS_FWD, s);
    (exact ? gsr_launch_loss_fwd_exact : gsr_launch_loss_fwd_fast)(s, W, H, C, image, target, C1, C2, h->d0.as<float>(),
                                                                          h->d1.as<float>(), h->d2.as<float>(), h->partial.as<float>());
    sc9.close();
    StageScope sc10(h->prof, ST_LOSS_BWD, s);
    (exact ? gsr_launch_loss_bwd_exact : gsr_launch_loss_bwd_fast)(s, W, H, C, image, target, lambda_dssim, h->d0.as<float>(),
                                                                          h->d1.as<float>(), h->d2.as<float>(), h->partial.as<float>(),
                                                                          loss_out, vpixels);
    sc10.close();
    HIPCHK(hipGetLastError());
    h->loss_vpixels = vpixels;
    h->loss_generation = h->generation;
    return GSR_OK;
}

int gsr_update_stats(gsr_handle* h, int32_t* max_radii, float* accum_grad_means2d, float* denom, void* stream) {
    if (!h || !max_radii || !accum_grad_means2d || !denom) return fail(GSR_E_INVALID_ARG, "null argument");
    if (!h->fwd_valid && h->dropped_by_reserve)
        return fail(GSR_E_STATE, "gsr_update_stats: a gsr_reserve that reallocated scratch (or gsr_drop_forward) dropped the "
                    "handle's last forward/backward pair");
    if (!h->fwd_valid || !h->bwd_valid) return fail(GSR_E_STATE, "gsr_update_stats needs a completed forward/backward pair");
    gsr_launch_update_stats((hipStream_t)stream, h->last_n, h->radii_cur, h->vmean2d_cur,
                            h->cfg.width, h->cfg.height, max_radii, accum_grad_means2d, denom);
    HIPCHK(hipGetLastError());
    return GSR_OK;
}

int gsr_profile_enable(gsr_handle* h, int on) {
    if (!h) return fail(GSR_E_INVALID_ARG, "null handle");
    h->prof.on = (on & 1) != 0;
    h->prof.ranges = (on & 2) != 0;
    if (!h->prof.on) h->prof.clear();
    return GSR_OK;
}

int gsr_profile_stages(gsr_handle* h, uint32_t stage_mask) {
    if (!h) return fail(GSR_E_INVALID_ARG, "null handle");
    h->prof.mask = stage_mask;
    return GSR_OK;
}

int gsr_profile_stage_count(void) { return ST_COUNT; }
const char* gsr_profile_stage_name(int stage) { return stage >= 0 && stage < ST_COUNT ? kStageNames[stage] : ""; }

int gsr_profile_read(gsr_handle* h, double* ms_sum, int* launches, int reset) {
    if (!h || !ms_sum || !launches) return fail(GSR_E_INVALID_ARG, "null argument");
    for (int i = 0; i < ST_COUNT; i++) { ms_sum[i] = 0.0; launches[i] = 0; }
    for (auto& r : h->prof.recs) {
        float ms = 0.0f;
        HIPCHK(hipEventSynchronize(r.b));
        HIPCHK(hipEventElapsedTime(&ms, r.a, r.b));
        ms_sum[r.stage] += ms;
        if (!r.extra) launches[r.stage] += 1;
    }
    if (reset) h->prof.clear();
    return GSR_OK;
}

int gsr_profile_read_intervals(gsr_handle* h, int stage, double* ms_out, int max_n, int* n_out) {
    if (!h || !n_out || (max_n > 0 && !ms_out)) return fail(GSR_E_INVALID_ARG, "null argument");
    if (stage < 0 || stage >= ST_COUNT) return fail(GSR_E_INVALID_ARG, "unknown stage %d", stage);
    int n = 0;
    hipEvent_t prev = nullptr;
    for (auto& r : h->prof.recs) {
        if (r.stage != stage || r.extra) continue;
        if (prev) {
            if (n < max_n) {
                float ms = 0.0f;
                HIPCHK(hipEventSynchronize(r.a));
                HIPCHK(hipEventElapsedTime(&ms, prev, r.a));
                ms_out[n] = ms;
            }
            n++;
        }
        prev = r.a;
    }
    *n_out = n;
    return GSR_OK;
}

int gsr_backward_trainer_tail(gsr_handle* h, const gsr_inputs* in, const gsr_camera* cam, const float* vpixels,
                              const gsr_tail_state* st, void* stream_v) {
    int rc = check_inputs(h, in, cam);
    if (rc) return rc;
    if (!vpixels || !st) return fail(GSR_E_INVALID_ARG, "null vpixels / tail state");
    if ((rc = check_backward_state(h, in, "gsr_backward_trainer_tail"))) return rc;
    if ((st->flags & ~GSR_GRADS_COLOR_COTANGENT) != 0u || st->reserved != 0u) return fail(GSR_E_INVALID_ARG, "unknown gsr_tail_state.flags / reserved bits");
    if (st->forward_generation != 0 && st->forward_generation != h->generation)
        return fail(GSR_E_STATE, "gsr_backward_trainer_tail for forward #%llu, but the handle's last forward is #%llu",
                    (unsigned long long)st->forward_generation, (unsigned long long)h->generation);
    if (st->scale_dims != 1 && st->scale_dims != 3) return fail(GSR_E_INVALID_ARG, "scale_dims must be 1 or 3");
    const int n = in->n, K = in->n_coeffs;
    if (n == 0) return GSR_OK;
    float lr_t[6];
    if ((rc = tail_lr_t(st->theta, st->mu, st->nu, st->lr, st->current_step, st->beta1, st->beta2, K == 1, lr_t)))
        return rc;
    if (in->means != st->theta[0] || in->rotations != st->theta[5] || in->shs != st->shs ||
        in->opacities != st->opacities_act || in->scales != st->scales_act)
        return fail(GSR_E_INVALID_ARG, "the inputs of the fused step must be the trainer's own arrays (means == theta[0], "
                    "rotations == theta[5], shs / opacities / scales == the activated copies)");
    if (((uintptr_t)st->theta[5] & 15) != 0) return fail(GSR_E_INVALID_ARG, "rotations must be 16-byte aligned");
    hipStream_t s = (hipStream_t)stream_v;
    const int C = h->cfg.mode;
    GsrCam k;
    if ((rc = composite_bwd_stage(h, s, in, cam, vpixels, st->vmeans2d, st->flags, &k))) return rc;
    StageScope sc12(h->prof, ST_PERGAUSS_BWD, s);
    const gsr::TailState S = gsr_make_tail_state(st->theta, st->mu, st->nu, lr_t, st->beta1, st->beta2, st->eps,
                                                 st->scale_dims, st->shs, st->opacities_act, st->scales_act);
    gsr_launch_pergauss_bwd_tail(s, n, K, in->sh_degree, C, k, geom_of(h), inst_of(h), h->vmean2d_cur, S,
                                 h->cfg.grad_precision == GSR_GRAD_FP32_REFERENCE, comp_of(h));
    sc12.close();
    HIPCHK(hipGetLastError());
    h->bwd_valid = true;
    h->inputs_consumed = true;
    return GSR_OK;
}

}
```

### gaussiansplatting.jl_amd/csrc/gsr_kernels.h

```cpp
#pragma once
#include <hip/hip_runtime.h>
#include <stdint.h>

#define GSR_TILE 16
#define GSR_BATCH 256
#define GSR_SORT_LDS_CAP 8192

struct GsrCam {
    float R[9];
    float t[3];
    float focal[2];
    float principal[2];
    float center[3];
    int width, height;
    int grid_x, grid_y;
    float near_plane, far_plane;
    int radius_clip;
    float blur_eps;
    int exact_cull;
    const float* R_dev;
    const float* t_dev;
};

struct GsrGeoRec { float4 q0, q1, q2, q3; };
constexpr uint32_t GSR_DENSE_RECT = 32;
struct GsrGeom {
    GsrGeoRec* rec;
    float4* normal;
    int32_t* radii;
    uint32_t* bsum;
    uint32_t* bpre;
};

struct GsrStream {
    float4* s0;
    float4* s1;
    float4* s2;
    float4* s3;
};

#define GSR_BWD_LONG_SEGS 32
#define GSR_ROW_F4(C) ((C) > 3 ? 4 : 3)
struct GsrInst {
    float4* rows;
};

enum GsrTotal {
    GSR_TOTAL_D = 0,
    GSR_TOTAL_MAX_LIST = 1,
    GSR_TOTAL_BIG = 2,
    GSR_TOTAL_MID4 = 3,
    GSR_TOTAL_VISIBLE = 4,
    GSR_TOTAL_SLOTS = 5,
    GSR_TOTAL_MID8 = 6,
    GSR_TOTAL_SEQ = 7,
    GSR_TOTAL_WORDS = 8
};
struct GsrTiles {
    uint32_t* start;
    uint32_t* count;
    uint32_t* order;
    uint32_t* ranges;
    uint32_t* tier_lists;
    uint32_t* totals;
    int n_tiles, grid_x;
};
struct GsrKeys { uint64_t* bins; uint32_t cap; const uint64_t* overflow ; };
struct GsrFrame {
    const float* background;
    float* image;
    uint32_t* n_contrib; float* final_T;
    uint32_t* values_sorted;
    uint8_t* covis; float* uncert;
};

int gsr_launch_preprocess(hipStream_t s, int n, int K, int degree, int channels, const float* means,
                          const float* scales, const float* rots, const float* opac, const float* shs, GsrCam cam,
                          GsrGeom geom, GsrTiles tiles, uint32_t* n_visible ,
                          GsrKeys keys , bool aggregating,
                          float* comp );
struct GsrBg8 { float v[8]; };
void gsr_launch_emit_compact(hipStream_t s, int n, GsrCam cam, GsrGeom geom, const uint32_t* tile_start, uint32_t* tile_fill,
                             uint64_t* keys, uint32_t max_list , uint32_t only_above);

inline size_t gsr_pose_partial_floats(int64_t n) { return n <= 0 ? 0 : (size_t)((n + 255) / 256) * 12; }
void gsr_launch_pergauss_bwd(hipStream_t s, int n, int K, int degree, int channels, const float* means,
                             const float* scales, const float* rots, const float* shs, GsrCam cam, GsrGeom geom,
                             GsrInst inst, float2* vmean2d, float* vmeans, float* vshs, float* vopac,
                             float* vscales, float* vrots, float* vR, float* vt ,
                             float* pose_part ,
                             float* vcolors ,
                             bool fp32_chain ,
                             const float* opac, const float* comp );
namespace gsr { struct TailState; }
void gsr_launch_pergauss_bwd_tail(hipStream_t s, int n, int K, int degree, int channels, GsrCam cam, GsrGeom geom,
                                  GsrInst inst, float2* vmean2d, const gsr::TailState& S, bool fp32_chain,
                                  const float* comp );
void gsr_launch_update_stats(hipStream_t s, int n, const int32_t* radii, const float2* vmean2d, int width, int height,
                             int32_t* max_radii, float* accum, float* denom);

void gsr_launch_sh_grad_views(hipStream_t s, int n, int K, int degree, int n_views, const float* centers,
                              const float* means, const float* vc_all, float* vshs);
void gsr_launch_sh_views_tail(hipStream_t s, int n, int K, int degree, int n_views, const float* centers,
                              const float* vc_all, const float* vmeans, const float* vopac_act, const float* vscales_act,
                              const float* vrot, const gsr::TailState& S);

void gsr_launch_tile_scan(hipStream_t s, GsrTiles tiles, GsrGeom geom, int n_blocks, const uint32_t* bvis,
                          uint32_t* host_mirror , uint32_t seq);
void gsr_launch_tile_sort(hipStream_t s, int channels, bool main_pass, GsrTiles tiles, GsrKeys keys, uint32_t n_mid4,
                          uint32_t n_mid8, uint32_t n_big, uint32_t first4, uint32_t first8,
                          uint64_t* big_scratch , size_t slab_stride,
                          GsrGeom geom, GsrStream stream, uint32_t* values_sorted);
void gsr_launch_tile_sort_mid(hipStream_t s, int channels, GsrTiles tiles, GsrKeys keys, uint32_t grid4, uint32_t grid8,
                              GsrGeom geom, GsrStream stream, uint32_t* values_sorted, uint32_t cap_instances);

void gsr_launch_fill_background(hipStream_t s, size_t n_pixels, int channels, GsrFrame frame);
struct GsrTierLists {
    const uint32_t* lists;
    uint32_t n_tiles, n_big, n_mid8, n_mid4;
    uint32_t split_len;
};
#define GSR_TIER_TILE(tile, tiers, slot)                                                                                       \
    do {                                                                                                                       \
        uint32_t b_ = (slot);                                                                                                  \
        const uint32_t* list_ = (tiers).lists;                                                               \
        if (b_ >= (tiers).n_big) { b_ -= (tiers).n_big; list_ = (tiers).lists + (tiers).n_tiles;             \
            if (b_ >= (tiers).n_mid8) { b_ -= (tiers).n_mid8; list_ = (tiers).lists + 2 * (size_t)(tiers).n_tiles; } }   \
        (tile) = (int)list_[b_];                                                                                               \
    } while (0)
void gsr_launch_composite_fwd(hipStream_t s, int channels, GsrCam cam, GsrTiles tiles, GsrStream stream, GsrFrame frame,
                              const GsrTierLists* only_listed );
void gsr_launch_sort_composite_fwd(hipStream_t s, int channels, GsrCam cam, GsrTiles tiles, GsrKeys keys, GsrGeom geom,
                                   GsrStream stream, GsrFrame frame, uint32_t cap_instances,
                                   bool keep_backward_state );
void gsr_launch_composite_bwd(hipStream_t s, int channels, GsrCam cam, GsrTiles tiles, GsrStream stream, GsrFrame frame,
                              const float* vpixels, GsrInst inst,
                              uint32_t split_len ,
                              bool color_only ,
                              bool accurate );
void gsr_launch_composite_bwd_listed(hipStream_t s, int channels, GsrCam cam, GsrTiles tiles, GsrTierLists tiers,
                                     GsrStream stream, GsrFrame frame, const float* vpixels, GsrInst inst,
                                     float* long_state );

#define GSR_ADAM_MAX_GROUPS 8
void gsr_launch_prologue_fwd(hipStream_t s, int n, int k_rest, int scale_dims, const float* sh_color,
                             const float* sh_remainder, const float* opacities, const float* scales, float* shs,
                             float* opacities_act, float* scales_act);
void gsr_launch_prologue_bwd(hipStream_t s, int n, int k_rest, int scale_dims, const float* opacities_act,
                             const float* scales_act, const float* vshs, const float* vopacities_act,
                             const float* vscales_act, float* v_sh_color, float* v_sh_remainder, float* v_opacities,
                             float* v_scales);
void gsr_launch_adam(hipStream_t s, int n_groups, float* const* theta, const float* const* grad, float* const* mu,
                     float* const* nu, const long long* count, const float* lr_t, float beta1, float beta2, float eps);

void gsr_launch_trainer_tail(hipStream_t s, int n, int k_rest, int scale_dims, const float* const* grads,
                             float* const* theta, float* const* mu, float* const* nu, const float* lr_t, float beta1,
                             float beta2, float eps, float* shs, float* opac_act, float* scales_act);
size_t gsr_findall_scratch_bytes(long long n);
void gsr_launch_findall(hipStream_t s, long long n, const uint8_t* mask, uint32_t* indices, uint32_t* count_dev,
                        uint32_t* scratch);
void gsr_launch_gather_rows(hipStream_t s, int n_groups, const void* const* src, void* const* dst, const int* row_words,
                            const uint32_t* idx, long long count);
void gsr_launch_triad(hipStream_t s, size_t n4, float* a, const float* b, const float* c, float q);

#define GSR_COMPOSE_MAX_GROUPS 24
void gsr_launch_grad_mean(hipStream_t s, long long n, const float* accum, const float* denom, float* out);
void gsr_launch_densify_mask(hipStream_t s, int kind, long long n, long long n_grad, const float* grad, const float* scales,
                             int scale_dims, const float* opacities, const int32_t* max_radii, float thr, float gamma,
                             float min_opacity, int max_screen_size, uint8_t* mask);
void gsr_launch_compose_rows(hipStream_t s, int n_groups, const void* const* src, void* const* dst, const int* row_words,
                             const int* new_zero, const uint32_t* keep_idx, long long n_keep, const uint32_t* sel_idx,
                             long long n_sel, int reps);
void gsr_launch_split_transform(hipStream_t s, long long n_new, int scale_dims, float* points, const float* rots,
                                float* scales, uint32_t seed);
void gsr_launch_reset_opacity(hipStream_t s, long long n, float* opacities);
void gsr_launch_morton_codes(hipStream_t s, long long n, const float* points, const float lo[3], const float inv_extent[3],
                             unsigned long long* codes);
void gsr_launch_nonfinite_scan(hipStream_t s, int n_groups, const float* const* src, const int* row_words, long long n_rows,
                               uint32_t* counts, uint32_t* first_bad);
void gsr_launch_ply_rows(hipStream_t s, bool pack, long long n, int kr, float* points, float* dc, float* rest, float* opac,
                         float* scales, float* rots, float* rows);

void gsr_launch_mcmc_weights(hipStream_t s, long long n, int scale_dims, const float* opac, const float* scales, float min_opacity,
                             float log_max_scale, uint32_t* q, uint8_t* dead);
size_t gsr_mcmc_sample_scratch_words(long long n);
void gsr_launch_mcmc_sample(hipStream_t s, long long n, const uint32_t* q, long long m, uint32_t seed, uint32_t* sampled,
                            int32_t* counts, unsigned long long* total, unsigned long long* scratch);
void gsr_launch_mcmc_split_sampled(hipStream_t s, long long n, int scale_dims, const int32_t* counts, const float* binoms, int n_max,
                                   float min_opacity, float* opac, float* scales);
void gsr_launch_mcmc_relocation_params(hipStream_t s, long long m, const float* o, const int32_t* ratio, const float* binoms,
                                       int n_max, float min_opacity, float* new_o, float* coeff);
void gsr_launch_mcmc_relocate_rows(hipStream_t s, int n_groups, void* const* x, const int* row_words, const int* new_zero,
                                   long long n, const uint32_t* dead, const uint32_t* sampled, long long m);
void gsr_launch_mcmc_inject_noise(hipStream_t s, long long n, int scale_dims, float* points, const float* opac, const float* scales,
                                  const float* rots, float lr, float max_kick, uint32_t seed);
size_t gsr_mcmc_regularization_scratch_floats(long long n);
void gsr_launch_mcmc_regularization(hipStream_t s, long long n, int scale_dims, const float* opac, const float* scales,
                                    float opacity_reg, float scale_reg, float* loss_out, float* vopac, float* vscales,
                                    float* scratch);

#define GSR_SSIM_DECL(SUF)                                                                                              \
    void gsr_launch_ssim_fwd_##SUF(hipStream_t s, int W, int H, int CH, int B, const float* img, const float* ref, float C1, \
                                   float C2, int train, float* ssim_map, float* d0, float* d1, float* d2);             \
    void gsr_launch_ssim_bwd_##SUF(hipStream_t s, int W, int H, int CH, int B, const float* img, const float* ref,      \
                                   const float* dL_dmap, const float* d0, const float* d1, const float* d2, float* dL_dimg); \
     \
    size_t gsr_loss_partial_pairs_##SUF(int W, int H);                                                                 \
    void gsr_launch_loss_fwd_##SUF(hipStream_t s, int W, int H, int C, const float* image, const float* target, float C1, \
                                   float C2, float* d0, float* d1, float* d2, float* partial);                         \
    void gsr_launch_loss_bwd_##SUF(hipStream_t s, int W, int H, int C, const float* image, const float* target, float lambda, \
                                   const float* d0, const float* d1, const float* d2, const float* partial, float* loss_out, \
                                   float* vpixels);
GSR_SSIM_DECL(exact)
GSR_SSIM_DECL(fast)
#undef GSR_SSIM_DECL

namespace gsr {
struct AdamHyper;
struct BilateralTv { float weight, nx, ny, nz, n12, rx, ry, rz; };
}
int gsr_bilateral_chunks(int W, int H, int gx, int gy);
size_t gsr_bilateral_partial_bytes(int W, int H, int gx, int gy, int gz);
void gsr_launch_bilateral_fwd(hipStream_t s, int W, int H, int C, const float* image, const float* grid, int gx, int gy,
                              int gz, float* out);
void gsr_launch_bilateral_bwd(hipStream_t s, int W, int H, int C, const float* image, const float* grid, int gx, int gy,
                              int gz, const float* vout, float* vimage, float* vgrid, float* partial);
void gsr_launch_bilateral_tv(hipStream_t s, int n, int gx, int gy, int gz, const float* grids, const gsr::BilateralTv& tv,
                             float* loss_out, float* grad_out, float* partial);
void gsr_launch_bilateral_adam_tail(hipStream_t s, int n, int gx, int gy, int gz, float* grids, float* mu, float* nu,
                                    const float* vgrid, int view, const gsr::BilateralTv& tv, const gsr::AdamHyper& h,
                                    float* tv_loss_out, float* partial);

size_t gsr_normal_loss_scratch_floats(int W, int H);
void gsr_launch_normal_loss_fwd(hipStream_t s, int W, int H, const float* image, const float* focal, const float* principal,
                                float weight, float* loss_out, float* stats_out, float* weights_out, float* scratch);
void gsr_launch_normal_loss_bwd(hipStream_t s, int W, int H, const float* image, const float* focal, const float* principal,
                                float weight, float* vpixels, const float* scratch);
size_t gsr_flatten_loss_scratch_floats(int64_t n);
void gsr_launch_flatten_loss(hipStream_t s, int n, int scale_dims, const float* scales, float weight, float* loss_out,
                             float* vscales, float* scratch);

size_t gsr_depth_loss_scratch_size(int W, int H);
void gsr_launch_depth_target(hipStream_t s, int W, int H, const float* prior, const float* anchor, float qstep, float* target_out,
                             float* half_band_out, uint8_t* flags_out);
void gsr_launch_depth_loss_fwd(hipStream_t s, int W, int H, int C, const float* image, const float* prior, const float* anchor,
                               float qstep, float lambda_grad, float weight, float* loss_out, float* stats_out, float* target_out,
                               float* half_band_out, uint8_t* flags_out, void* scratch);
void gsr_launch_depth_loss_bwd(hipStream_t s, int W, int H, int C, const float* image, float lambda_grad, float weight,
                               float* vpixels, const void* scratch);

size_t gsr_sky_scratch_size(int W, int H);
void gsr_launch_sky_composite_fwd(hipStream_t s, int W, int H, int C, const float* image, const float* sky_rgb,
                                  const float* sky_weight, float loss_weight, float* out, float* loss_out, void* scratch);
void gsr_launch_sky_composite_bwd(hipStream_t s, int W, int H, int C, const float* image, const float* sky_rgb,
                                  const float* sky_weight, float loss_weight, float* vpixels, float* vsky, const void* scratch);

size_t gsr_eval_scratch_size(int W, int H);
void gsr_launch_eval_metrics(hipStream_t s, int W, int H, int C, const float* image, const float* sky_rgb,
                             const float* target_f32, const unsigned char* target_u8, int quantize, float* ssim_map, float* out,
                             void* scratch);
void gsr_launch_frame_rgb8(hipStream_t s, int W, int H, int C, const float* image, const float* sky_rgb, int flip_rows,
                           unsigned char* rgb8_out);

size_t gsr_knn_scratch_size(long long n);
void gsr_launch_knn_scales(hipStream_t s, long long n, const float* points, const int32_t* order, float point_size,
                           int scale_dims, float* scales_out, float* dist2_out, void* scratch);

size_t gsr_filter3d_scratch_size(long long n);
void gsr_launch_filter3d_compute(hipStream_t s, long long n, const float* points, int n_cameras, const float* cams,
                                 float near_plane, float k, float* filter, uint8_t* seen, uint32_t* count, void* scratch);
void gsr_launch_filter3d_apply(hipStream_t s, long long n, const float* opac, const float* scales, const float* filter, int raw,
                               float* opac_out, float* scales_out);
void gsr_launch_filter3d_apply_bwd(hipStream_t s, long long n, const float* opac, const float* scales, const float* filter,
                                   const float* g_opac, const float* g_scales, float* v_opac, float* v_scales);

struct GsrTsdfGrid {
    int nx, ny, nz;
    float o[3];
    float h;
};
struct GsrTsdfCam {
    float R[9];
    float t[3];
    float fx, fy, cx, cy;
};
size_t gsr_mesh_scratch_size(int nx, int ny, int nz);
void gsr_launch_tsdf_integrate(hipStream_t s, const GsrTsdfGrid& g, const GsrTsdfCam& c, int W, int H, int C, const float* image,
                               float min_alpha, float near_plane, float trunc, float* volume, float* color);
void gsr_launch_mesh_count(hipStream_t s, const GsrTsdfGrid& g, const float* volume, uint32_t* counts, void* scratch);
// ... 3 lines not shown
```

### gaussiansplatting.jl_amd/csrc/gsr_policy.cpp

```cpp
#include "../../include/gsr.h"

#include <algorithm>
#include <cstdlib>
#include <cstring>

#include "agg_plan.h"

namespace {

constexpr int kTile = 16;
constexpr uint64_t kBinsBudgetMin = 512ull << 20, kBinsBudgetPerInstance = 160ull;
constexpr uint32_t kHybridMinCap = 1024u;
constexpr uint32_t kTunerMaxAge = 4096u;

inline uint64_t round64_slack(uint64_t v) { return (v + v / 4 + 63) & ~63ull; }
inline uint64_t budget_of(uint64_t configured, uint64_t instances) {
    return configured ? configured : std::max<uint64_t>(kBinsBudgetMin, kBinsBudgetPerInstance * instances);
}

uint32_t bins_capacity_after(uint64_t instances, uint64_t longest, uint64_t tiles, uint64_t budget_bytes) {
    const uint64_t mean_list = instances / tiles + 1;
    const uint64_t budget = budget_of(budget_bytes, instances);
    const uint64_t cap = (budget / (8ull * (tiles + 1))) & ~63ull;
    uint64_t want = std::max<uint64_t>(64ull, round64_slack(longest));
// ... 45 lines not shown
    cfg->preprocess_form = preprocess_form < 0 ? -1 : (preprocess_form != 0 ? 1 : 0);
    cfg->form_tuner = 1;
    cfg->beside_max_tiles = 0xFFFFFFFFu;
    cfg->bwd_split_max_tiles = 256u;
    cfg->agg_max_bands = gsr_agg::kMaxBandsDefault;
}

void gsr_policy_state_init(gsr_policy_state* st) {
    if (!st) return;
    memset(st, 0, sizeof *st);
    st->tuner.form = -1;
}

uint32_t gsr_bins_capacity_after(int64_t n_rendered, int32_t max_tile_instances, int32_t width, int32_t height,
                                 uint64_t bins_budget_bytes, uint32_t current_capacity) {
    if (n_rendered < 0 || max_tile_instances < 0 || width <= 0 || height <= 0) return 0u;
    const uint64_t tiles = (uint64_t)((width + kTile - 1) / kTile) * (uint64_t)((height + kTile - 1) / kTile);
    return bins_capacity_next((uint64_t)n_rendered, (uint64_t)max_tile_instances, tiles, bins_budget_bytes, current_capacity);
}

void gsr_policy_agg_plan(int32_t grid_x, int32_t grid_y, uint32_t max_pos, int32_t* n_bands, int32_t* band_rows,
                         size_t* lds_bytes, int32_t* words16) {
    if (grid_x <= 0 || grid_y <= 0) return;
    const gsr_agg::Plan p = gsr_agg::plan(grid_x, grid_y, max_pos);
    if (n_bands) *n_bands = p.n_bands;
    if (band_rows) *band_rows = p.band_rows;
    if (lds_bytes) *lds_bytes = p.lds;
    if (words16) *words16 = p.w32 ? 1 : 0;
}

int32_t gsr_policy_preprocess_form(const gsr_policy_config* cfg, int32_t form_request, int32_t n, uint32_t bin_cap_view,
                                   int32_t skewed) {
    if (!cfg || n <= 0) return GSR_FORM_DIRECT;
    return form_for(cfg, form_request, n, bin_cap_view, skewed != 0);
}

int32_t gsr_policy_form_is_open(const gsr_policy_config* cfg, int32_t n, uint32_t bin_cap_view) {
    return cfg && form_is_open(cfg, n, bin_cap_view) ? 1 : 0;
}

void gsr_policy_begin_view(const gsr_policy_config* cfg, gsr_policy_state* st, int32_t n, const float* timed_ms,
                           gsr_view_plan* plan) {
    memset(plan, 0, sizeof *plan);
    plan->timed_slot = -1;
    st->views++;
    const uint64_t T = tiles_of(cfg);
    const uint64_t nn = n > 0 ? (uint64_t)n : 1ull;
    if (st->bin_cap == 0 && !st->compact_sticky) {
        const uint64_t est = 8ull * nn / T + 64;
        st->bin_cap = (uint32_t)((est < (1u << 20) ? est : (1u << 20)) + 63) & ~63u;
    }
    const uint64_t budget = budget_of(cfg->bins_budget_bytes, (uint64_t)st->last_n_rendered);
    const uint64_t cap_budget = (budget / (8ull * (T + 1))) & ~63ull;
    if (st->bin_cap > cap_budget) st->bin_cap = (uint32_t)cap_budget;
    const bool use_bins = st->bin_cap >= 64u;
    st->bin_cap_view = plan->bin_cap_view = use_bins ? st->bin_cap : 0u;

    int request = cfg->preprocess_form;
    if (request < 0 && cfg->form_tuner && form_is_open(cfg, n, plan->bin_cap_view)) {
        gsr_form_tuner& t = st->tuner;
        const bool decided = t.phase == GSR_TUNER_TIMED_VIEWS + 1;
        if (decided && (++t.age > kTunerMaxAge || std::abs(n - t.n_ref) > t.n_ref / 4)) {
            t.phase = 0; t.form = -1; t.age = 0;
            st->tuner_rearms++;
        }
        if (t.phase == GSR_TUNER_TIMED_VIEWS + 1) {
            request = t.form;
        } else if (st->views > 2) {
            if (t.phase == GSR_TUNER_TIMED_VIEWS) {
                if (timed_ms) {
                    t.ms[0] = std::min(timed_ms[0], timed_ms[2]);
                    t.ms[1] = std::min(timed_ms[1], timed_ms[3]);
                    t.form = t.ms[1] < 0.97f * t.ms[0] ? 1 : 0;
                    t.phase = GSR_TUNER_TIMED_VIEWS + 1; t.n_ref = n; t.age = 0;
                    request = t.form;
                    plan->tuner_decided = 1;
                }
            } else {
                plan->timed_slot = t.phase;
                request = t.phase & 1;
                t.phase++;
            }
        }
    }
    plan->skewed = st->last_n_rendered > 0 && (uint64_t)st->last_max_tile * T > 6ull * (uint64_t)st->last_n_rendered;
    plan->form_request = request;
    plan->form = n > 0 ? form_for(cfg, request, n, plan->bin_cap_view, plan->skewed != 0) : GSR_FORM_DIRECT;
    const uint64_t prev_tiers = (uint64_t)st->tier_n[0] + st->tier_n[1] + st->tier_n[2];
    plan->hold_fused = prev_tiers > 0 && prev_tiers <= cfg->beside_max_tiles;
    const auto guess = [&](uint32_t prev) -> uint32_t {
        if (!prev) return 0u;
        const uint64_t g = (uint64_t)prev + prev / 4 + 16u, T = tiles_of(cfg);
        return (uint32_t)(g < T ? g : T);
    };
    const bool spec_sorts = plan->hold_fused && plan->bin_cap_view > 0;
    plan->spec_mid4 = spec_sorts ? guess(st->tier_n[0]) : 0u;
    plan->spec_mid8 = spec_sorts ? guess(st->tier_n[1]) : 0u;
}

void gsr_policy_end_view(const gsr_policy_config* cfg, gsr_policy_state* st, const gsr_view_plan* plan, int64_t n_rendered,
                         uint32_t max_tile_instances, uint32_t n_mid4, uint32_t n_mid8, uint32_t n_big,
                         uint64_t cap_instances, int32_t fused_allowed, gsr_view_outcome* out) {
    memset(out, 0, sizeof *out);
    const uint64_t T = tiles_of(cfg);
    const uint64_t D = n_rendered > 0 ? (uint64_t)n_rendered : 0ull;
    const bool use_bins = plan->bin_cap_view > 0;
    const bool overflow = use_bins && max_tile_instances > plan->bin_cap_view;
    const bool hybrid = overflow && plan->bin_cap_view >= kHybridMinCap;
    const bool compact = !use_bins || (overflow && !hybrid);
    out->binning = compact ? GSR_BINNING_COMPACT : (hybrid ? GSR_BINNING_OVERFLOW : GSR_BINNING_BINS);
    const uint32_t want = bins_capacity_next(D, max_tile_instances, T, cfg->bins_budget_bytes, use_bins ? st->bin_cap : 0u);
    if (want == 0u) {
        st->bin_cap = 0; st->compact_sticky = 1;
    } else if (want > st->bin_cap || !use_bins) {
        out->bins_regrown = use_bins && want > st->bin_cap;
        st->bin_cap = want; st->compact_sticky = 0;
    }
    out->bin_cap_next = st->bin_cap;
    const bool spec = fused_allowed != 0 && use_bins;
    const bool held = spec && plan->hold_fused != 0;
    out->fused_done = spec && D <= cap_instances && !(overflow && !hybrid);
    out->long_tiles = (n_mid4 | n_mid8 | n_big) != 0u;
    const uint64_t tiers = (uint64_t)n_mid4 + n_mid8 + n_big;
    out->beside = held && out->fused_done && out->long_tiles && tiers <= cfg->beside_max_tiles;
    out->launch_fused_now = held && !out->beside && out->fused_done;
    const bool spec_sorted = (plan->spec_mid4 | plan->spec_mid8) != 0u && D <= cap_instances && max_tile_instances <= plan->bin_cap_view;
    out->sorted_mid4 = spec_sorted ? (plan->spec_mid4 < n_mid4 ? plan->spec_mid4 : n_mid4) : 0u;
    out->sorted_mid8 = spec_sorted ? (plan->spec_mid8 < n_mid8 ? plan->spec_mid8 : n_mid8) : 0u;
    if (!use_bins) st->compact_views++;
    else if (overflow && !hybrid) st->compact_fallbacks++;
    else if (hybrid) st->overflow_views++;
    if (out->bins_regrown) st->bins_regrowths++;
    if (spec && !held && D > cap_instances) st->fused_relaunches++;
    if (held) st->held_views++;
    st->last_n_rendered = (int64_t)D;
    st->last_max_tile = max_tile_instances;
    st->tier_n[0] = n_mid4; st->tier_n[1] = n_mid8; st->tier_n[2] = n_big;
}

void gsr_policy_bwd_split(const gsr_policy_config* cfg, uint32_t n_mid4, uint32_t n_mid8, uint32_t n_big, gsr_bwd_split* out) {
    memset(out, 0, sizeof *out);
    const uint32_t cut[3] = {8192u, 4096u, 1024u};
    const uint32_t have[3] = {n_big, n_mid8, n_mid4};
    uint32_t* take[3] = {&out->n_big, &out->n_mid8, &out->n_mid4};
    uint64_t n = 0;
    out->split_len = 0xFFFFFFFFu;
    for (int t = 0; t < 3 && n + have[t] <= cfg->bwd_split_max_tiles; t++) {
        n += *take[t] = have[t];
        out->split_len = cut[t];
    }
    if (n == 0) out->split_len = 0xFFFFFFFFu;
}

}
```

### gaussiansplatting.jl_amd/csrc/gsr_sizes.h

```cpp
#pragma once
#include <cstddef>
#include <cstdint>

struct gsr_gaussian_bytes {
    size_t geo;
    size_t radii;
    size_t block;
    size_t gnormal;
    size_t vmean2d;
    size_t pose_part;
    size_t comp;
};

inline gsr_gaussian_bytes gsr_sizes_per_gaussian(size_t n, int C, size_t pose_partial_floats, bool antialiased = false) {
    const size_t nn = n > 0 ? n : 1;
    gsr_gaussian_bytes b;
    b.geo = nn * 64;
    b.radii = nn * 4;
    b.block = ((n + 255) / 256 + 1) * 4;
    b.gnormal = C > 5 ? nn * 16 : 0;
    b.vmean2d = n * 8;
    b.pose_part = pose_partial_floats * 4;
    b.comp = antialiased ? nn * 4 : 0;
    return b;
}

struct gsr_instance_bytes {
    size_t values_sorted;
    size_t stream;
    size_t s3;
    size_t rows;
};

inline gsr_instance_bytes gsr_sizes_per_instance(uint64_t D, uint64_t D_slots, int C) {
    gsr_instance_bytes b;
    b.values_sorted = (size_t)D * 4;
    b.stream = (size_t)D * 16;
    b.s3 = C > 3 ? (size_t)D * 16 : 0;
    b.rows = (size_t)D_slots * 64;
    return b;
}

inline gsr_instance_bytes gsr_sizes_reserve_instances(uint64_t D, int C) {
    gsr_instance_bytes b = gsr_sizes_per_instance(D, 3 * D, C);
    b.rows /= 2;
    return b;
}
```

### gaussiansplatting.jl_amd/csrc/pergauss.hip

```cpp
#include "gsr_kernels.h"
#include "gsr_dispatch.h"
#include "tile_mask.h"
#include "wave_reduce.h"
#include "adam_math.h"
#include "splat_math.h"
#include "sh_rows.h"

namespace {
using namespace gsr::splat;
using gsr::dispatch_bool;
using gsr::dispatch_degree;
using gsr::store_sh_rows;
using gsr::tail_sh_group;

constexpr uint32_t DENSE_RECT = GSR_DENSE_RECT;

__device__ __forceinline__ M33 add33(const M33& a, const M33& b) {
    M33 o;
#pragma unroll
    for (int i = 0; i < 3; i++)
#pragma unroll
        for (int j = 0; j < 3; j++) o.m[i][j] = a.m[i][j] + b.m[i][j];
    return o;
}
// ... 190 lines not shown
            float part[16];
#pragma unroll
            for (int k = 0; k < 16; k++) part[k] = 0.0f;
            for (uint32_t k = lane; k < a; k += 64) {
                const uint32_t tx = sx0 + k % sw, ty = sy0 + k / sw;
                if (cam.exact_cull && !tile_may_touch(smx, smy, sa, sb, sc, stau, (int)tx * GSR_TILE, (int)ty * GSR_TILE))
                    continue;
                const float4* row = inst.rows + (size_t)GSR_ROW_F4(channels) * (o + k);
                const float4 f0 = row[0], f1 = row[1], f2 = row[2];
                part[0] += f0.x; part[1] += f0.y; part[2] += f0.z; part[3] += f0.w;
                part[4] += f1.x; part[5] += f1.y; part[6] += f1.z; part[7] += f1.w;
                part[8] += f2.x; part[9] += f2.y;
                if (channels > 5) {
                    const float4 f3 = row[3];
                    part[10] += f2.z; part[11] += f2.w; part[12] += f3.x;
                }
            }
            const float total = gsr::wave_reduce_transposed<13>(part, lb);
            if (gsr::wave_reduce_writer(lane)) bounce[wave][slot] = total;
            __builtin_amdgcn_wave_barrier();
            if (lane == src) {
#pragma unroll
                for (int k = 0; k < 13; k++) acc[k] = bounce[wave][k];
            }
            __builtin_amdgcn_wave_barrier();
        }
    }
}

struct ProjectBwd {
    float mc[3];
    M33 Rg, M;
    float qn[4], inv_norm;
    float vmean[3];
    M33 vSigma;
};
template <bool AA>
__device__ __forceinline__ ProjectBwd project_bwd(const GsrCam& cam, const M33& R, const float t[3], const float p[3],
                                                  const float4 q4, const float s[3], const GsrGeoRec& rec, const float4 a1,
                                                  const float2 vm2, float rho, float vrho, int channels, bool with_pose,
                                                  float poseR[9], float poset[3]) {
    ProjectBwd o;
    const float4 g0 = rec.q0, g1 = rec.q1;
    M22 Ci, vCi;
    Ci.m[0][0] = g0.z; Ci.m[1][0] = g0.w; Ci.m[0][1] = g0.w; Ci.m[1][1] = g1.x;
    vCi.m[0][0] = a1.x; vCi.m[1][0] = a1.y; vCi.m[0][1] = a1.y; vCi.m[1][1] = a1.z;
    M22 nC;
#pragma unroll
    for (int a = 0; a < 2; a++)
#pragma unroll
        for (int b = 0; b < 2; b++) nC.m[a][b] = -Ci.m[a][b];
    M22 vS2 = mul22(mul22(nC, vCi), Ci);
    if constexpr (AA) {
        const float dc = Ci.m[0][0] * Ci.m[1][1] - Ci.m[0][1] * Ci.m[1][0];
        const float vsq = 0.5f * vrho / (rho + 1e-6f);
        const float ct = 1.0f - rho * rho;
        vS2.m[0][0] = vS2.m[0][0] + vsq * (ct * Ci.m[0][0] - cam.blur_eps * dc);
        vS2.m[1][0] = vS2.m[1][0] + vsq * ct * Ci.m[1][0];
        vS2.m[0][1] = vS2.m[0][1] + vsq * ct * Ci.m[0][1];
        vS2.m[1][1] = vS2.m[1][1] + vsq * (ct * Ci.m[1][1] - cam.blur_eps * dc);
    }
    to_camera(R, t, p, o.mc);
    const float* mc = o.mc;
    const ForwardChain fc = forward_chain(R, mc, q4, s, cam);
    o.Rg = fc.Rg; o.M = fc.M; o.inv_norm = fc.inv_norm;
#pragma unroll
    for (int k = 0; k < 4; k++) o.qn[k] = fc.qn[k];
    const M33& Sigma = fc.Sigma;
    const M33& Sc = fc.Sc;
    const Persp& pr = fc.pr;
    const float rz = pr.rz, rz2 = rz * rz, rz3 = rz2 * rz;
    const float* f = cam.focal;
    float JtV[3][2];
#pragma unroll
    for (int a = 0; a < 3; a++)
#pragma unroll
        for (int b = 0; b < 2; b++) JtV[a][b] = pr.J[0][a] * vS2.m[0][b] + pr.J[1][a] * vS2.m[1][b];
    M33 vSc;
#pragma unroll
    for (int a = 0; a < 3; a++)
#pragma unroll
        for (int b = 0; b < 3; b++) vSc.m[a][b] = JtV[a][0] * pr.J[0][b] + JtV[a][1] * pr.J[1][b];
    float A[2][3], B[2][3], vJ[2][3];
#pragma unroll
    for (int a = 0; a < 2; a++)
#pragma unroll
        for (int b = 0; b < 3; b++) {
            A[a][b] = vS2.m[a][0] * pr.J[0][b] + vS2.m[a][1] * pr.J[1][b];
            B[a][b] = vS2.m[0][a] * pr.J[0][b] + vS2.m[1][a] * pr.J[1][b];
        }
#pragma unroll
    for (int a = 0; a < 2; a++)
#pragma unroll
        for (int b = 0; b < 3; b++) {
            float u = A[a][0] * Sc.m[b][0] + A[a][1] * Sc.m[b][1] + A[a][2] * Sc.m[b][2];
            float v = B[a][0] * Sc.m[0][b] + B[a][1] * Sc.m[1][b] + B[a][2] * Sc.m[2][b];
            vJ[a][b] = u + v;
        }
    float vx = f[0] * rz * vm2.x;
    float vy = f[1] * rz * vm2.y;
    float vz = -rz2 * (f[0] * mc[0] * vm2.x + f[1] * mc[1] * vm2.y);
    float rx = mc[0] * rz, ry = mc[1] * rz;
    if (-pr.lim_neg[0] <= rx && rx <= pr.lim[0]) vx += -f[0] * rz2 * vJ[0][2];
    else vz += -f[0] * rz3 * vJ[0][2] * pr.txy[0];
    if (-pr.lim_neg[1] <= ry && ry <= pr.lim[1]) vy += -f[1] * rz2 * vJ[1][2];
    else vz += -f[1] * rz3 * vJ[1][2] * pr.txy[1];
    vz += -f[0] * rz2 * vJ[0][0] - f[1] * rz2 * vJ[1][1] + 2.0f * f[0] * pr.txy[0] * rz3 * vJ[0][2] +
          2.0f * f[1] * pr.txy[1] * rz3 * vJ[1][2];
    float vmc[3] = {vx, vy, vz};
    if (channels > 3) vmc[2] = vmc[2] + a1.w;
#pragma unroll
    for (int c = 0; c < 3; c++) o.vmean[c] = R.m[0][c] * vmc[0] + R.m[1][c] * vmc[1] + R.m[2][c] * vmc[2];
    o.vSigma = mul33(mul33(tr33(R), vSc), R);
    if (with_pose) {
        M33 vR0;
#pragma unroll
        for (int r = 0; r < 3; r++)
#pragma unroll
            for (int c = 0; c < 3; c++) vR0.m[r][c] = vmc[r] * p[c];
        M33 u = mul33(mul33(vSc, R), tr33(Sigma));
        M33 v = mul33(mul33(tr33(vSc), R), Sigma);
        M33 vR2 = add33(add33(vR0, u), v);
#pragma unroll
        for (int r = 0; r < 3; r++) {
#pragma unroll
            for (int c = 0; c < 3; c++) poseR[c * 3 + r] = fabsf(vR2.m[r][c]) > 1e-7f ? vR2.m[r][c] : 0.0f;
            poset[r] = fabsf(vmc[r]) > 1e-7f ? vmc[r] : 0.0f;
        }
    }
    return o;
}

__device__ __forceinline__ void normal_bwd(int channels, const float acc[16], const M33& R, const M33& Rg, const float s[3],
                                           const float mc[3], M33& vRg) {
#pragma unroll
    for (int a = 0; a < 3; a++)
#pragma unroll
        for (int b = 0; b < 3; b++) vRg.m[a][b] = 0.0f;
    if (channels > 5) {
        const float4 a2 = make_float4(acc[10], acc[11], acc[12], 0.0f);
        float nn[3]; int k; float sg;
        gaussian_normal(R, Rg, s, mc, nn, k, sg);
#pragma unroll
        for (int r = 0; r < 3; r++) {
            float g = R.m[0][r] * a2.x + R.m[1][r] * a2.y + R.m[2][r] * a2.z;
            float v = sg * g;
            vRg.m[r][0] = k == 0 ? v : 0.0f;
            vRg.m[r][1] = k == 1 ? v : 0.0f;
            vRg.m[r][2] = k == 2 ? v : 0.0f;
        }
    }
}

template <int DEG>
__device__ __forceinline__ void sh_bwd(const float* sh, const float p[3], const GsrCam& cam, const float vc[3], float b[16],
                                       float vmsh[3]) {
    float d0[3], dir[3];
    view_dir(p, cam.center, d0, dir);
    sh_basis<DEG>(dir, b);
    float dcx[3] = {0, 0, 0}, dcy[3] = {0, 0, 0}, dcz[3] = {0, 0, 0};
    if (DEG > 0) {
        const float x = dir[0], y = dir[1], z = dir[2];
#pragma unroll
        for (int c = 0; c < 3; c++) {
            dcx[c] = -SH1 * sh_coeff(sh, 3, c); dcy[c] = -SH1 * sh_coeff(sh, 1, c); dcz[c] = SH1 * sh_coeff(sh, 2, c);
        }
        if (DEG > 1) {
            float x2 = x * x, y2 = y * y, z2 = z * z, xy = x * y, xz = x * z, yz = y * z;
#pragma unroll
            for (int c = 0; c < 3; c++) {
                dcx[c] = dcx[c] + SH2C1 * y * sh_coeff(sh, 4, c) + SH2C3 * 2.0f * -x * sh_coeff(sh, 6, c) +
                         SH2C4 * z * sh_coeff(sh, 7, c) + SH2C5 * 2.0f * x * sh_coeff(sh, 8, c);
                dcy[c] = dcy[c] + SH2C1 * x * sh_coeff(sh, 4, c) + SH2C2 * z * sh_coeff(sh, 5, c) +
                         SH2C3 * 2.0f * -y * sh_coeff(sh, 6, c) + SH2C5 * 2.0f * -y * sh_coeff(sh, 8, c);
                dcz[c] = dcz[c] + SH2C2 * y * sh_coeff(sh, 5, c) + SH2C3 * 4.0f * z * sh_coeff(sh, 6, c) +
                         SH2C4 * x * sh_coeff(sh, 7, c);
            }
            if (DEG > 2) {
#pragma unroll
                for (int c = 0; c < 3; c++) {
                    dcx[c] = dcx[c] + SH3C1 * sh_coeff(sh, 9, c) * 3.0f * 2.0f * xy + SH3C2 * sh_coeff(sh, 10, c) * yz +
                             SH3C3 * sh_coeff(sh, 11, c) * -2.0f * xy + SH3C4 * sh_coeff(sh, 12, c) * -3.0f * 2.0f * xz +
                             SH3C5 * sh_coeff(sh, 13, c) * (-3.0f * x2 + 4.0f * z2 - y2) +
                             SH3C6 * sh_coeff(sh, 14, c) * 2.0f * xz + SH3C7 * sh_coeff(sh, 15, c) * 3.0f * (x2 - y2);
                    dcy[c] = dcy[c] + SH3C1 * sh_coeff(sh, 9, c) * 3.0f * (x2 - y2) + SH3C2 * sh_coeff(sh, 10, c) * xz +
                             SH3C3 * sh_coeff(sh, 11, c) * (-3.0f * y2 + 4.0f * z2 - x2) +
                             SH3C4 * sh_coeff(sh, 12, c) * -3.0f * 2.0f * yz + SH3C5 * sh_coeff(sh, 13, c) * -2.0f * xy +
                             SH3C6 * sh_coeff(sh, 14, c) * -2.0f * yz + SH3C7 * sh_coeff(sh, 15, c) * -3.0f * 2.0f * xy;
                    dcz[c] = dcz[c] + SH3C2 * sh_coeff(sh, 10, c) * xy + SH3C3 * sh_coeff(sh, 11, c) * 4.0f * 2.0f * yz +
                             SH3C4 * sh_coeff(sh, 12, c) * 3.0f * (2.0f * z2 - x2 - y2) +
                             SH3C5 * sh_coeff(sh, 13, c) * 4.0f * 2.0f * xz + SH3C6 * sh_coeff(sh, 14, c) * (x2 - y2);
                }
            }
        }
    }
    float vdir[3];
    vdir[0] = dcx[0] * vc[0] + dcx[1] * vc[1] + dcx[2] * vc[2];
    vdir[1] = dcy[0] * vc[0] + dcy[1] * vc[1] + dcy[2] * vc[2];
    vdir[2] = dcz[0] * vc[0] + dcz[1] * vc[1] + dcz[2] * vc[2];
    float s2 = d0[0] * d0[0] + d0[1] * d0[1] + d0[2] * d0[2];
    float inv_s = 1.0f / sqrtf(s2 * s2 * s2);
    vmsh[0] = ((s2 - d0[0] * d0[0]) * vdir[0] - d0[1] * d0[0] * vdir[1] - d0[2] * d0[0] * vdir[2]) * inv_s;
    vmsh[1] = (-d0[0] * d0[1] * vdir[0] + (s2 - d0[1] * d0[1]) * vdir[1] - d0[2] * d0[1] * vdir[2]) * inv_s;
    vmsh[2] = (-d0[0] * d0[2] * vdir[0] - d0[1] * d0[2] * vdir[1] + (s2 - d0[2] * d0[2]) * vdir[2]) * inv_s;
}

template <bool FUSED>
__device__ __forceinline__ void store_or_apply_sh(int i, int n, int K, float* __restrict__ vshs, const float* vcolors,
                                                  const gsr::TailState& TS, const float f_b[16], const float f_vc[3],
                                                  int f_nb, const float f_vmean[3], float f_vopac, const float f_vs[3],
                                                  const float f_vq[4]) {
    __shared__ float tail_b[256][17];
    __shared__ float tail_vc[256][3];
    __shared__ int tail_nb[256];
    const int i0 = blockIdx.x * 256;
    const int cnt = min(256, n - i0);
    const int K3 = 3 * K;
    if (FUSED || !vcolors) {
#pragma unroll
        for (int k = 0; k < 16; k++) tail_b[threadIdx.x][k] = f_b[k];
#pragma unroll
        for (int c = 0; c < 3; c++) tail_vc[threadIdx.x][c] = f_vc[c];
        tail_nb[threadIdx.x] = f_nb;
    }
    if constexpr (!FUSED) {
        if (!vcolors) {
            __syncthreads();
            store_sh_rows(vshs, i0, cnt, K3, [&](int il, int j) {
                const int k = j / 3, c = j - 3 * k;
                return k < tail_nb[il] ? tail_b[il][k] * tail_vc[il][c] : 0.0f;
            });
        }
    }
    if constexpr (FUSED) {
        if (i < n) gsr::tail_gauss_apply(TS, i, f_vmean, f_vopac, f_vs, f_vq);
        __syncthreads();
        auto grad = [&](int il, int k, int c) { return k < tail_nb[il] ? tail_b[il][k] * tail_vc[il][c] : 0.0f; };
        auto sh_group = [&](float* __restrict__ th, float* __restrict__ mu, float* __restrict__ nu, int R, int k0,
                            const gsr::AdamHyper& hy) { tail_sh_group(TS, i0, cnt, K3, th, mu, nu, R, k0, hy, grad); };
        sh_group(TS.dc, TS.dc_mu, TS.dc_nu, 3, 0, TS.h_dc);
        if (K > 1) sh_group(TS.rest, TS.rest_mu, TS.rest_nu, 3 * (K - 1), 1, TS.h_rest);
    }
}

template <int DEG, bool FUSED, bool F32CHAIN = false, bool AA = false>
__global__ __launch_bounds__(256, 1) void pergauss_bwd_kernel(int n, int K, int channels, const float* __restrict__ means,
                                                           const float* __restrict__ scales,
                                                           const float4* __restrict__ rots,
                                                           const float* __restrict__ shs, GsrCam cam, GsrGeom geom,
                                                           GsrInst inst, float2* __restrict__ vmean2d_out,
                                                           float* __restrict__ vmeans,
                                                           float* __restrict__ vshs, float* __restrict__ vopac,
                                                           float* __restrict__ vscales, float4* __restrict__ vrots,
                                                           float* __restrict__ pose_part,
                                                           float* __restrict__ vcolors, gsr::TailState TS,
                                                           const float* __restrict__ opac,
                                                           const float* __restrict__ comp) {
    const int i = blockIdx.x * 256 + threadIdx.x;
    float poseR[9] = {0, 0, 0, 0, 0, 0, 0, 0, 0}, poset[3] = {0, 0, 0};
    GsrGeoRec rec;
    rec.q0 = rec.q1 = rec.q2 = rec.q3 = make_float4(0.0f, 0.0f, 0.0f, 0.0f);
    float p_in[3] = {0, 0, 0}, s_in[3] = {0, 0, 0};
    float4 q_in = make_float4(1.0f, 0.0f, 0.0f, 0.0f);
    int radius_in = 0;
    float o_in = 0.0f, rho_in = 0.0f;
    if (i < n) {
        radius_in = geom.radii[i];
        rec = geom.rec[i];
        const float* mp = FUSED ? TS.points : means;
        const float* sp = FUSED ? TS.scales_act : scales;
        const float4* qp = FUSED ? reinterpret_cast<const float4*>(TS.rots) : rots;
        p_in[0] = mp[3 * i]; p_in[1] = mp[3 * i + 1]; p_in[2] = mp[3 * i + 2];
        s_in[0] = sp[3 * i]; s_in[1] = sp[3 * i + 1]; s_in[2] = sp[3 * i + 2];
        q_in = qp[i];
        if constexpr (AA) {
            o_in = FUSED ? TS.opac_act[i] : opac[i];
            rho_in = comp[i];
        }
    }
    const bool visible = radius_in > 0;
    float acc[16];
    sum_gradient_rows(i, visible, rec, geom, cam, inst, channels, acc);

    float f_vmean[3] = {0, 0, 0}, f_vs[3] = {0, 0, 0}, f_vq[4] = {0, 0, 0, 0}, f_vopac = 0.0f;
    float f_vc[3] = {0, 0, 0}, f_b[16];
    int f_nb = 0;
#pragma unroll
    for (int k = 0; k < 16; k++) f_b[k] = 0.0f;
    if (i < n) {
        if (!visible) {
            vmean2d_out[i] = make_float2(0.0f, 0.0f);
            if constexpr (!FUSED) {
#pragma unroll
                for (int c = 0; c < 3; c++) { vmeans[3 * i + c] = 0.0f; vscales[3 * i + c] = 0.0f; }
                vrots[i] = make_float4(0, 0, 0, 0);
                vopac[i] = 0.0f;
                if (vcolors) { vcolors[3 * i] = 0.0f; vcolors[3 * i + 1] = 0.0f; vcolors[3 * i + 2] = 0.0f; }
            }
        } else {
            const float4 a0 = make_float4(acc[0], acc[1], acc[2], acc[3]);
            const float4 a1 = make_float4(acc[4], acc[5], acc[6], acc[7]);
            const float2 vm2 = make_float2(acc[8], acc[9]);
            vmean2d_out[i] = vm2;
            const float vo = AA ? a0.w * rho_in : a0.w, vrho = AA ? a0.w * o_in : 0.0f;
            if constexpr (FUSED) f_vopac = vo; else vopac[i] = vo;
            M33 R; float t[3];
            load_pose(cam, R, t);
            const float p[3] = {p_in[0], p_in[1], p_in[2]};
            const float4 q4 = q_in;
            const float s[3] = {s_in[0], s_in[1], s_in[2]};
            const ProjectBwd pb = project_bwd<AA>(cam, R, t, p, q4, s, rec, a1, vm2, rho_in, vrho, channels, pose_part != nullptr,
                                                  poseR, poset);
            M33 vRg;
            normal_bwd(channels, acc, R, pb.Rg, s, pb.mc, vRg);
            float vs[3], vq[4];
            if constexpr (!F32CHAIN) {
                scales_rots_bwd_f64<AA>(cam, R, t, p, q4, s, a1.x, a1.y, a1.z, vRg, rho_in, vrho, vs, vq);
            } else {
                M33 S;
#pragma unroll
                for (int a = 0; a < 3; a++)
#pragma unroll
                    for (int b = 0; b < 3; b++) S.m[a][b] = 0.0f;
                S.m[0][0] = s[0]; S.m[1][1] = s[1]; S.m[2][2] = s[2];
                M33 vM = mul33(add33(pb.vSigma, tr33(pb.vSigma)), pb.M);
                M33 vRq = add33(mul33(vM, S), vRg);
#pragma unroll
                for (int c = 0; c < 3; c++)
                    vs[c] = pb.Rg.m[0][c] * vM.m[0][c] + pb.Rg.m[1][c] * vM.m[1][c] + pb.Rg.m[2][c] * vM.m[2][c];
                unnorm_quat2rot_bwd<float>(vRq.m, pb.qn, pb.inv_norm, vq);
            }
            if constexpr (FUSED) {
#pragma unroll
                for (int k = 0; k < 4; k++) f_vq[k] = vq[k];
#pragma unroll
                for (int c = 0; c < 3; c++) f_vs[c] = vs[c];
            } else {
                vrots[i] = make_float4(vq[0], vq[1], vq[2], vq[3]);
#pragma unroll
                for (int c = 0; c < 3; c++) vscales[3 * i + c] = vs[c];
            }

            const float* sh = FUSED ? TS.rest + (size_t)3 * (K - 1) * i : shs + (size_t)3 * K * i + 3;
            const uint32_t clamp_bits = __float_as_uint(rec.q2.y);
            float vc[3] = {a0.x * (1.0f - (float)(clamp_bits & 1u)), a0.y * (1.0f - (float)((clamp_bits >> 1) & 1u)),
                           a0.z * (1.0f - (float)((clamp_bits >> 2) & 1u))};
            float b[16], vmsh[3];
            sh_bwd<DEG>(sh, p, cam, vc, b, vmsh);
            constexpr int NB = (DEG + 1) * (DEG + 1);
            if (!FUSED && vcolors) {
                vcolors[3 * i] = vc[0]; vcolors[3 * i + 1] = vc[1]; vcolors[3 * i + 2] = vc[2];
            } else {
                f_nb = NB;
#pragma unroll
                for (int c = 0; c < 3; c++) f_vc[c] = vc[c];
#pragma unroll
                for (int k = 0; k < NB; k++) f_b[k] = b[k];
            }
#pragma unroll
            for (int c = 0; c < 3; c++) {
                if constexpr (FUSED) f_vmean[c] = pb.vmean[c] + vmsh[c]; else vmeans[3 * i + c] = pb.vmean[c] + vmsh[c];
            }
        }
    }
    store_or_apply_sh<FUSED>(i, n, K, vshs, vcolors, TS, f_b, f_vc, f_nb, f_vmean, f_vopac, f_vs, f_vq);
    if (pose_part) {
        __shared__ float pose_red[4][12];
#pragma unroll
        for (int k = 0; k < 12; k++) {
            float v = k < 9 ? poseR[k] : poset[k - 9];
#pragma unroll
            for (int off = 32; off > 0; off >>= 1) v += __shfl_xor(v, off);
            if ((threadIdx.x & 63) == 0) pose_red[threadIdx.x >> 6][k] = v;
        }
        __syncthreads();
        if (threadIdx.x < 12) {
            const int k = threadIdx.x;
            pose_part[(size_t)blockIdx.x * 12 + k] = pose_red[0][k] + pose_red[1][k] + pose_red[2][k] + pose_red[3][k];
        }
    }
}

__global__ __launch_bounds__(256) void pose_final_kernel(int n_part, const float* __restrict__ part, float* __restrict__ vR,
                                                         float* __restrict__ vt) {
    __shared__ double red[12][256];
    double s[12];
#pragma unroll
    for (int k = 0; k < 12; k++) s[k] = 0.0;
    for (int i = threadIdx.x; i < n_part; i += 256)
#pragma unroll
        for (int k = 0; k < 12; k++) s[k] += (double)part[(size_t)i * 12 + k];
#pragma unroll
    for (int k = 0; k < 12; k++) red[k][threadIdx.x] = s[k];
    __syncthreads();
    if (threadIdx.x >= 12) return;
    const int k = threadIdx.x;
    double t = 0.0;
    for (int i = 0; i < 256; i++) t += red[k][i];
    if (k < 9) vR[k] = (float)t; else vt[k - 9] = (float)t;
}

__global__ __launch_bounds__(256) void update_stats_kernel(int n, const int32_t* __restrict__ radii,
                                                           const float2* __restrict__ vmean2d, float res_x,
                                                           float res_y, int32_t* __restrict__ max_radii,
                                                           float* __restrict__ accum, float* __restrict__ denom) {
    const int i = blockIdx.x * 256 + threadIdx.x;
    if (i >= n) return;
    const int r = radii[i];
    if (!(r > 0)) return;
    max_radii[i] = max(max_radii[i], r);
    const float2 g = vmean2d[i];
    const float gx = g.x * res_x * 0.5f, gy = g.y * res_y * 0.5f;
    accum[i] += sqrtf(gx * gx + gy * gy);
    denom[i] += 1.0f;
}

}

void gsr_launch_update_stats(hipStream_t s, int n, const int32_t* radii, const float2* vmean2d, int width, int height,
                             int32_t* max_radii, float* accum, float* denom) {
    if (n <= 0) return;
    hipLaunchKernelGGL(update_stats_kernel, dim3((n + 255) / 256), dim3(256), 0, s, n, radii, vmean2d, (float)width,
                       (float)height, max_radii, accum, denom);
}

void gsr_launch_pergauss_bwd(hipStream_t s, int n, int K, int degree, int channels, const float* means,
                             const float* scales, const float* rots, const float* shs, GsrCam cam, GsrGeom geom,
                             GsrInst inst, float2* vmean2d, float* vmeans, float* vshs, float* vopac,
                             float* vscales, float* vrots, float* vR, float* vt, float* pose_part, float* vcolors,
                             bool fp32_chain, const float* opac, const float* comp) {
    if (n <= 0) return;
    dim3 grid((n + 255) / 256), block(256);
    const float4* r4 = reinterpret_cast<const float4*>(rots);
    float4* vr4 = reinterpret_cast<float4*>(vrots);
    const gsr::TailState none{};
    dispatch_degree(degree, [&](auto d) {
        constexpr int DEG = d;
        dispatch_bool(fp32_chain, [&](auto f) {
            constexpr bool F32 = f;
            dispatch_bool(comp != nullptr, [&](auto a) {
                constexpr bool AA = a;
                hipLaunchKernelGGL((pergauss_bwd_kernel<DEG, false, F32, AA>), grid, block, 0, s, n, K, channels, means, scales,
                                   r4, shs, cam, geom, inst, vmean2d, vmeans, vshs, vopac, vscales, vr4,
                                   vR ? pose_part : nullptr, vcolors, none, opac, comp);
            });
        });
    });
    if (vR) hipLaunchKernelGGL(pose_final_kernel, dim3(1), dim3(256), 0, s, (int)grid.x, pose_part, vR, vt);
}

void gsr_launch_pergauss_bwd_tail(hipStream_t s, int n, int K, int degree, int channels, GsrCam cam, GsrGeom geom,
                                  GsrInst inst, float2* vmean2d, const gsr::TailState& S, bool fp32_chain, const float* comp) {
    if (n <= 0) return;
    dim3 grid((n + 255) / 256), block(256);
    const float4* r4 = reinterpret_cast<const float4*>(S.rots);
    float* const no_f = nullptr;
    dispatch_degree(degree, [&](auto d) {
        constexpr int DEG = d;
        dispatch_bool(fp32_chain, [&](auto f) {
            constexpr bool F32 = f;
            dispatch_bool(comp != nullptr, [&](auto a) {
                constexpr bool AA = a;
                hipLaunchKernelGGL((pergauss_bwd_kernel<DEG, true, F32, AA>), grid, block, 0, s, n, K, channels, S.points,
                                   S.scales_act, r4, (const float*)nullptr, cam, geom, inst, vmean2d, no_f, no_f, no_f, no_f,
                                   (float4*)nullptr, no_f, no_f, S, (const float*)nullptr, comp);
            });
        });
    });
}
```

### gaussiansplatting.jl_amd/csrc/sh_rows.h

```cpp
#pragma once
#include <stdint.h>
#include "adam_math.h"

namespace gsr {

template <class Grad>
__device__ __forceinline__ void tail_sh_group(const gsr::TailState& TS, int i0, int cnt, int K3, float* __restrict__ th,
                                              float* __restrict__ mu, float* __restrict__ nu, int R, int k0,
                                              const gsr::AdamHyper& hy, Grad grad) {
    const size_t base = (size_t)i0 * R;
    const int total = cnt * R;
    const uint32_t inv = (1u << 20) / (uint32_t)R + 1u;
    th += base; mu += base; nu += base;
    const bool aligned = ((((uintptr_t)th) | ((uintptr_t)mu) | ((uintptr_t)nu)) & 15) == 0;
    const int total4 = aligned ? total >> 2 : 0;
    auto element = [&](int e, float& t, float& m, float& v) {
        const int il = (int)(((uint32_t)e * inv) >> 20);
        const int j = e - il * R;
        const int kb = j / 3, c = j - 3 * kb, k = k0 + kb;
        const float g = grad(il, k, c);
        t = gsr::adam_update(t, g, m, v, hy);
        TS.shs[(size_t)(i0 + il) * K3 + 3 * k0 + j] = t;
    };
    for (int f = threadIdx.x; f < total4; f += 256) {
        float4 t4 = reinterpret_cast<float4*>(th)[f], m4 = reinterpret_cast<float4*>(mu)[f],
               v4 = reinterpret_cast<float4*>(nu)[f];
        element(4 * f, t4.x, m4.x, v4.x);
        element(4 * f + 1, t4.y, m4.y, v4.y);
        element(4 * f + 2, t4.z, m4.z, v4.z);
        element(4 * f + 3, t4.w, m4.w, v4.w);
        reinterpret_cast<float4*>(th)[f] = t4;
        reinterpret_cast<float4*>(mu)[f] = m4;
        reinterpret_cast<float4*>(nu)[f] = v4;
    }
    for (int e = 4 * total4 + threadIdx.x; e < total; e += 256) {
        float t = th[e], m = mu[e], v = nu[e];
        element(e, t, m, v);
        th[e] = t; mu[e] = m; nu[e] = v;
    }
}

template <class Value>
__device__ __forceinline__ void store_sh_rows(float* __restrict__ vshs, int i0, int cnt, int K3, Value value) {
    const uint32_t inv = (1u << 20) / (uint32_t)K3 + 1u;
    float* __restrict__ dst = vshs + (size_t)i0 * K3;
    const int total = cnt * K3;
    auto element = [&](int e) {
        const int il = (int)(((uint32_t)e * inv) >> 20);
        return value(il, e - il * K3);
    };
    const int total4 = (((uintptr_t)dst & 15) == 0) ? total >> 2 : 0;
    for (int f = threadIdx.x; f < total4; f += 256)
        reinterpret_cast<float4*>(dst)[f] = make_float4(element(4 * f), element(4 * f + 1), element(4 * f + 2), element(4 * f + 3));
    for (int e = 4 * total4 + threadIdx.x; e < total; e += 256) dst[e] = element(e);
}

}
```

### gaussiansplatting.jl_amd/csrc/splat_math.h

```cpp
#pragma once
#include "gsr_kernels.h"

namespace gsr::splat {

constexpr float SH0 = 0.28209479177387814f;
constexpr float SH1 = 0.4886025119029199f;
constexpr float SH2C1 = 1.0925484305920792f;
constexpr float SH2C2 = -1.0925484305920792f;
constexpr float SH2C3 = 0.31539156525252005f;
constexpr float SH2C4 = -1.0925484305920792f;
constexpr float SH2C5 = 0.5462742152960396f;
constexpr float SH3C1 = -0.5900435899266435f;
constexpr float SH3C2 = 2.890611442640554f;
constexpr float SH3C3 = -0.4570457994644658f;
constexpr float SH3C4 = 0.3731763325901154f;
constexpr float SH3C5 = -0.4570457994644658f;
constexpr float SH3C6 = 1.445305721320277f;
constexpr float SH3C7 = -0.5900435899266435f;

struct M33 { float m[3][3]; };
struct M22 { float m[2][2]; };

__device__ __forceinline__ M33 mul33(const M33& a, const M33& b) {
    M33 o;
#pragma unroll
    for (int i = 0; i < 3; i++)
#pragma unroll
        for (int j = 0; j < 3; j++) o.m[i][j] = a.m[i][0] * b.m[0][j] + a.m[i][1] * b.m[1][j] + a.m[i][2] * b.m[2][j];
    return o;
}
__device__ __forceinline__ M33 tr33(const M33& a) {
    M33 o;
#pragma unroll
    for (int i = 0; i < 3; i++)
#pragma unroll
        for (int j = 0; j < 3; j++) o.m[i][j] = a.m[j][i];
    return o;
}

__device__ __forceinline__ void load_pose(const GsrCam& cam, M33& R, float t[3]) {
    const bool dev = cam.R_dev != nullptr;
#pragma unroll
    for (int r = 0; r < 3; r++)
#pragma unroll
        for (int c = 0; c < 3; c++) {
            const float host = cam.R[r * 3 + c];
            R.m[r][c] = dev ? cam.R_dev[c * 3 + r] : host;
        }
#pragma unroll
    for (int k = 0; k < 3; k++) t[k] = cam.t_dev ? cam.t_dev[k] : cam.t[k];
}

__device__ __forceinline__ M33 quat2rot(const float4 q4, float qn[4], float& inv_norm) {
    float n2 = q4.x * q4.x + q4.y * q4.y + q4.z * q4.z + q4.w * q4.w;
    inv_norm = 1.0f / sqrtf(n2);
    float w = q4.x * inv_norm, x = q4.y * inv_norm, y = q4.z * inv_norm, z = q4.w * inv_norm;
    qn[0] = w; qn[1] = x; qn[2] = y; qn[3] = z;
    float x2 = x * x, y2 = y * y, z2 = z * z, xy = x * y, xz = x * z, yz = y * z, wx = w * x, wy = w * y, wz = w * z;
    M33 R;
    R.m[0][0] = 1.0f - 2.0f * (y2 + z2); R.m[1][0] = 2.0f * (xy + wz); R.m[2][0] = 2.0f * (xz - wy);
    R.m[0][1] = 2.0f * (xy - wz); R.m[1][1] = 1.0f - 2.0f * (x2 + z2); R.m[2][1] = 2.0f * (yz + wx);
    R.m[0][2] = 2.0f * (xz + wy); R.m[1][2] = 2.0f * (yz - wx); R.m[2][2] = 1.0f - 2.0f * (x2 + y2);
    return R;
}

__device__ __forceinline__ M33 cov3d(const M33& Rg, const float s[3], M33& M) {
#pragma unroll
    for (int r = 0; r < 3; r++)
#pragma unroll
        for (int c = 0; c < 3; c++) M.m[r][c] = Rg.m[r][c] * s[c];
    return mul33(M, tr33(M));
}

struct Persp {
    float lim[2], lim_neg[2], txy[2], rz;
    float J[2][3];
};
__device__ __forceinline__ Persp persp_common(const float mc[3], const GsrCam& cam) {
    Persp p;
    const int res[2] = {cam.width, cam.height};
    p.rz = 1.0f / mc[2];
    float rz2 = p.rz * p.rz;
#pragma unroll
    for (int k = 0; k < 2; k++) {
        float tan_fov = (0.5f * (float)res[k]) / cam.focal[k];
        float stf = 0.3f * tan_fov;
        float pp = cam.principal[k] * (float)res[k];
        p.lim[k] = ((float)res[k] - pp) / cam.focal[k] + stf;
        p.lim_neg[k] = pp / cam.focal[k] + stf;
        float v = mc[k] * p.rz;
        float c = fmaxf(-p.lim_neg[k], v);
        c = fminf(p.lim[k], c);
        p.txy[k] = mc[2] * c;
    }
    p.J[0][0] = cam.focal[0] * p.rz; p.J[1][0] = 0.0f;
    p.J[0][1] = 0.0f;                p.J[1][1] = cam.focal[1] * p.rz;
    p.J[0][2] = -cam.focal[0] * p.txy[0] * rz2;
    p.J[1][2] = -cam.focal[1] * p.txy[1] * rz2;
    return p;
}


template <int DEG>
__device__ __forceinline__ void sh_basis(const float d[3], float b[16]) {
    float x = d[0], y = d[1], z = d[2];
    b[0] = SH0;
    if (DEG > 0) {
        b[1] = -SH1 * y; b[2] = SH1 * z; b[3] = -SH1 * x;
    }
    if (DEG > 1) {
        float x2 = x * x, y2 = y * y, z2 = z * z, xy = x * y, xz = x * z, yz = y * z;
        b[4] = SH2C1 * xy; b[5] = SH2C2 * yz; b[6] = SH2C3 * (2.0f * z2 - x2 - y2);
        b[7] = SH2C4 * xz; b[8] = SH2C5 * (x2 - y2);
        if (DEG > 2) {
            b[9] = SH3C1 * y * (3.0f * x2 - y2);
            b[10] = SH3C2 * xy * z;
            b[11] = SH3C3 * y * (4.0f * z2 - x2 - y2);
            b[12] = SH3C4 * z * (2.0f * z2 - 3.0f * x2 - 3.0f * y2);
            b[13] = SH3C5 * x * (4.0f * z2 - x2 - y2);
            b[14] = SH3C6 * z * (x2 - y2);
            b[15] = SH3C7 * x * (x2 - 3.0f * y2);
        }
    }
}

__device__ __forceinline__ void gaussian_normal(const M33& Rw, const M33& Rg, const float s[3], const float mc[3],
                                                float n[3], int& k, float& sign) {
    k = (s[0] <= s[1] && s[0] <= s[2]) ? 0 : (s[1] <= s[2]) ? 1 : 2;
    const float m0 = k == 0 ? 1.0f : 0.0f, m1 = k == 1 ? 1.0f : 0.0f, m2 = k == 2 ? 1.0f : 0.0f;
    float ax[3];
#pragma unroll
    for (int r = 0; r < 3; r++) ax[r] = m0 * Rg.m[r][0] + m1 * Rg.m[r][1] + m2 * Rg.m[r][2];
    float nc[3];
#pragma unroll
    for (int r = 0; r < 3; r++) nc[r] = Rw.m[r][0] * ax[0] + Rw.m[r][1] * ax[1] + Rw.m[r][2] * ax[2];
    float d = nc[0] * mc[0] + nc[1] * mc[1] + nc[2] * mc[2];
    sign = d > 0.0f ? -1.0f : 1.0f;
#pragma unroll
    for (int r = 0; r < 3; r++) n[r] = sign * nc[r];
}

__device__ __forceinline__ void view_dir(const float p[3], const float* center, float d0[3], float dir[3]) {
    d0[0] = p[0] - center[0]; d0[1] = p[1] - center[1]; d0[2] = p[2] - center[2];
    const float inv = 1.0f / sqrtf(d0[0] * d0[0] + d0[1] * d0[1] + d0[2] * d0[2]);
    dir[0] = d0[0] * inv; dir[1] = d0[1] * inv; dir[2] = d0[2] * inv;
}

}
```

### include/gsr_policy.h

```cpp
#ifndef GSR_POLICY_H
#define GSR_POLICY_H

#include <stddef.h>
#include <stdint.h>

#ifdef __cplusplus
extern "C" {
#endif

#ifndef GSR_API
#define GSR_API __attribute__((visibility("default")))
#endif

enum {
    GSR_FORM_DIRECT = 0,
    GSR_FORM_AGG_W64 = 1,
    GSR_FORM_AGG_W32 = 2,
    GSR_FORM_AGG_BANDED = 3
};

enum {
    GSR_BINNING_BINS = 0,
    GSR_BINNING_COMPACT = 1,
    GSR_BINNING_OVERFLOW = 2
};

typedef struct gsr_form_tuner {
    int32_t phase;
    int32_t form;
    int32_t n_ref;
    uint32_t age;
    float ms[2];
} gsr_form_tuner;
#define GSR_TUNER_TIMED_VIEWS 4

typedef struct gsr_policy_config {
    int32_t grid_x, grid_y;
    uint64_t bins_budget_bytes;
    int32_t preprocess_form;
    int32_t form_tuner;
    uint32_t beside_max_tiles;
    uint32_t bwd_split_max_tiles;
    int32_t agg_max_bands;
    int32_t reserved;
} gsr_policy_config;

typedef struct gsr_policy_state {
    uint32_t bin_cap;
    uint32_t compact_sticky;
    int32_t last_n;
    uint32_t last_max_tile;
    int64_t last_n_rendered;
    uint32_t tier_n[3];
    uint32_t bin_cap_view;
    uint64_t views;
    gsr_form_tuner tuner;
    uint32_t bins_regrowths;
    uint32_t compact_fallbacks;
    uint32_t compact_views;
    uint32_t overflow_views;
    uint32_t tuner_rearms;
    uint32_t fused_relaunches;
    uint32_t held_views;
    uint32_t reserved;
} gsr_policy_state;

typedef struct gsr_view_plan {
    uint32_t bin_cap_view;
    int32_t form_request;
    int32_t form;
    int32_t timed_slot;
    int32_t skewed;
    int32_t hold_fused;
    int32_t tuner_decided;
    uint32_t spec_mid4, spec_mid8;
    int32_t reserved;
} gsr_view_plan;

typedef struct gsr_view_outcome {
    int32_t binning;
    int32_t fused_done;
    int32_t long_tiles;
    int32_t beside;
    int32_t launch_fused_now;
    int32_t reserved;
    uint32_t sorted_mid4, sorted_mid8;
    uint32_t bin_cap_next;
    uint32_t bins_regrown;
} gsr_view_outcome;

typedef struct gsr_bwd_split {
    uint32_t n_big, n_mid8, n_mid4;
    uint32_t split_len;
} gsr_bwd_split;

GSR_API void gsr_policy_config_init(gsr_policy_config* cfg, int32_t width, int32_t height, uint64_t bins_budget_bytes,
                                    int32_t preprocess_form);
GSR_API void gsr_policy_state_init(gsr_policy_state* st);

GSR_API void gsr_policy_agg_plan(int32_t grid_x, int32_t grid_y, uint32_t max_pos, int32_t* n_bands, int32_t* band_rows,
                                 size_t* lds_bytes, int32_t* words16);
GSR_API int32_t gsr_policy_preprocess_form(const gsr_policy_config* cfg, int32_t form_request, int32_t n, uint32_t bin_cap_view,
                                           int32_t skewed);
GSR_API int32_t gsr_policy_form_is_open(const gsr_policy_config* cfg, int32_t n, uint32_t bin_cap_view);

GSR_API void gsr_policy_begin_view(const gsr_policy_config* cfg, gsr_policy_state* st, int32_t n,
                                   const float* timed_ms , gsr_view_plan* plan);
GSR_API void gsr_policy_end_view(const gsr_policy_config* cfg, gsr_policy_state* st, const gsr_view_plan* plan,
                                 int64_t n_rendered, uint32_t max_tile_instances, uint32_t n_mid4, uint32_t n_mid8,
                                 uint32_t n_big, uint64_t cap_instances, int32_t fused_allowed, gsr_view_outcome* out);

GSR_API void gsr_policy_bwd_split(const gsr_policy_config* cfg, uint32_t n_mid4, uint32_t n_mid8, uint32_t n_big,
                                  gsr_bwd_split* out);

#ifdef __cplusplus
}
#endif
#endif
```

Before: 1604.

## Piggyback SH direction-Jacobian and culled-row zeroing onto composite backward launch

```diff
diff --git a/gaussiansplatting.jl_amd/_lib.py b/gaussiansplatting.jl_amd/_lib.py
--- a/gaussiansplatting.jl_amd/_lib.py
+++ b/gaussiansplatting.jl_amd/_lib.py
@@ -146,8 +146,13 @@
     _fields_ = [("n_big", C.c_uint32), ("n_mid8", C.c_uint32), ("n_mid4", C.c_uint32), ("split_len", C.c_uint32)]
 
 
+class BwdRowJob(C.Structure):
+    _fields_ = [("n_wg", C.c_uint32), ("slice", C.c_uint32)]
+
+
 POLICY_EXPORTS = ["gsr_policy_config_init", "gsr_policy_state_init", "gsr_policy_agg_plan", "gsr_policy_preprocess_form",
-                  "gsr_policy_form_is_open", "gsr_policy_begin_view", "gsr_policy_end_view", "gsr_policy_bwd_split"]
+                  "gsr_policy_form_is_open", "gsr_policy_begin_view", "gsr_policy_end_view", "gsr_policy_bwd_split",
+                  "gsr_policy_bwd_row_job"]
 
 
 def bind_policy(lib):
@@ -169,6 +174,8 @@
     lib.gsr_policy_end_view.restype = None
     lib.gsr_policy_bwd_split.argtypes = [P(PolicyConfig), C.c_uint32, C.c_uint32, C.c_uint32, P(BwdSplit)]
     lib.gsr_policy_bwd_split.restype = None
+    lib.gsr_policy_bwd_row_job.argtypes = [P(PolicyConfig), C.c_int32, P(BwdRowJob)]
+    lib.gsr_policy_bwd_row_job.restype = None
     lib.gsr_bins_capacity_after.argtypes = [C.c_int64, C.c_int32, C.c_int32, C.c_int32, C.c_uint64, C.c_uint32]
     lib.gsr_bins_capacity_after.restype = C.c_uint32
     return lib
diff --git a/gaussiansplatting.jl_amd/csrc/bwd_row_job.h b/gaussiansplatting.jl_amd/csrc/bwd_row_job.h
--- /dev/null
+++ b/gaussiansplatting.jl_amd/csrc/bwd_row_job.h
@@ -0,0 +1,49 @@
+#pragma once
+#include "splat_math.h"
+
+namespace gsr {
+
+template <int DEG>
+__device__ __forceinline__ void bwd_row_job_slice(const GsrRowJob& job, uint32_t w, int lane) {
+    using namespace gsr::splat;
+    const int K3 = 3 * job.K;
+    const int64_t begin = (int64_t)w * job.slice;
+    const int end = (int)(begin + job.slice < (int64_t)job.n ? begin + job.slice : (int64_t)job.n);
+    for (int base = (int)begin; base < end; base += 64) {
+        const int i = base + lane;
+        const bool mine = i < end;
+        const bool visible = mine && job.radii[i] > 0;
+        if (DEG > 0 && visible) {
+            const float p[3] = {job.means[3 * (size_t)i], job.means[3 * (size_t)i + 1], job.means[3 * (size_t)i + 2]};
+            float d0[3], dir[3], dcx[3], dcy[3], dcz[3];
+            view_dir(p, job.center, d0, dir);
+            sh_dir_jacobian<DEG>(job.shs + (size_t)K3 * i + 3, dir, dcx, dcy, dcz);
+            float* j9 = job.jac + 9 * (size_t)i;
+#pragma unroll
+            for (int c = 0; c < 3; c++) { j9[c] = dcx[c]; j9[3 + c] = dcy[c]; j9[6 + c] = dcz[c]; }
+        }
+        if (mine && !visible) {
+#pragma unroll
+            for (int c = 0; c < 3; c++) { job.vmeans[3 * (size_t)i + c] = 0.0f; job.vscales[3 * (size_t)i + c] = 0.0f; }
+            job.vrots[i] = make_float4(0.0f, 0.0f, 0.0f, 0.0f);
+            job.vopac[i] = 0.0f;
+        }
+        unsigned long long culled = __builtin_amdgcn_ballot_w64(mine && !visible);
+        while (culled) {
+            const int src = __builtin_ctzll(culled);
+            culled &= culled - 1ull;
+            if (lane < K3) job.vshs[(size_t)K3 * (base + src) + lane] = 0.0f;
+        }
+    }
+}
+
+__device__ __forceinline__ void bwd_row_job_run(const GsrRowJob& job, uint32_t w, int lane) {
+    switch (job.degree) {
+        case 0: bwd_row_job_slice<0>(job, w, lane); break;
+        case 1: bwd_row_job_slice<1>(job, w, lane); break;
+        case 2: bwd_row_job_slice<2>(job, w, lane); break;
+        default: bwd_row_job_slice<3>(job, w, lane); break;
+    }
+}
+
+}
diff --git a/gaussiansplatting.jl_amd/csrc/composite.hip b/gaussiansplatting.jl_amd/csrc/composite.hip
--- a/gaussiansplatting.jl_amd/csrc/composite.hip
+++ b/gaussiansplatting.jl_amd/csrc/composite.hip
@@ -307,6 +307,7 @@
     static_assert(!(C == 3 && BG0), ":rgb on a zero background is composite_bwd_kernel_rgb_bg0");
 #include "composite_bwd_body.inc"
 }
+__device__ void bwd_row_job(const GsrRowJob& job, uint32_t w, int lane);
 __global__ __attribute__((amdgpu_flat_work_group_size(1, 64), amdgpu_waves_per_eu(6, 6)))
 void composite_bwd_kernel_rgb_bg0(int W, int H, int grid_x,
                                                  const uint32_t* __restrict__ tile_start,
@@ -315,9 +316,13 @@
                                                  const float* __restrict__ vpixels,
                                                  const uint32_t* __restrict__ n_contrib,
                                                  const float* __restrict__ final_T, GsrInst inst,
-                                                 GsrTierLists tiers) {
+                                                 GsrTierLists tiers, GsrRowJob job) {
     constexpr int C = 3, VC = 3;
     constexpr bool BG0 = true, ACC = false;
+    if (blockIdx.x >= job.first_wg) {
+        bwd_row_job(job, blockIdx.x - job.first_wg, (int)threadIdx.x);
+        return;
+    }
 #include "composite_bwd_body.inc"
 }
 
@@ -498,9 +503,11 @@
     });
 }
 
-void gsr_launch_composite_bwd(hipStream_t s, int channels, GsrCam cam, GsrTiles tiles, GsrStream stream, GsrFrame frame,
-                              const float* vpixels, GsrInst inst, uint32_t split_len, bool color_only, bool accurate) {
+bool gsr_launch_composite_bwd(hipStream_t s, int channels, GsrCam cam, GsrTiles tiles, GsrStream stream, GsrFrame frame,
+                              const float* vpixels, GsrInst inst, const GsrRowJob* job, uint32_t split_len, bool color_only,
+                              bool accurate) {
     dim3 grid(cam.grid_x * cam.grid_y), block(64);
+    bool carried = false;
     Bg bg = make_bg(frame.background, channels);
     GsrTierLists none{};
     none.split_len = split_len;
@@ -511,9 +518,13 @@
 #define LAUNCH2(CC, ZZ) do { if (accurate) LAUNCH_K(CC, false, CC, true); else LAUNCH_K(CC, ZZ, CC, false); } while (0)
 #define LAUNCH3(CC, ZZ) do { if (accurate) LAUNCH_K(CC, false, 3, true); else LAUNCH_K(CC, ZZ, 3, false); } while (0)
     if (channels == 3) {
-        if (bg0 && !accurate)
-            hipLaunchKernelGGL(composite_bwd_kernel_rgb_bg0, grid, block, 0, s, cam.width, cam.height, cam.grid_x, tiles.start, tiles.order,
-                               stream, bg, vpixels, frame.n_contrib, frame.final_T, inst, none);
+        if (bg0 && !accurate) {
+            GsrRowJob j{};
+            if (job && job->n > 0 && job->n_wg > 0) { j = *job; carried = true; }
+            j.first_wg = grid.x;
+            hipLaunchKernelGGL(composite_bwd_kernel_rgb_bg0, dim3(grid.x + j.n_wg), block, 0, s, cam.width, cam.height, cam.grid_x,
+                               tiles.start, tiles.order, stream, bg, vpixels, frame.n_contrib, frame.final_T, inst, none, j);
+        }
         else LAUNCH2(3, false);
     }
     else if (color_only) {
@@ -525,6 +536,7 @@
 #undef LAUNCH_K
 #undef LAUNCH2
 #undef LAUNCH3
+    return carried;
 }
 
 void gsr_launch_composite_bwd_listed(hipStream_t s, int channels, GsrCam cam, GsrTiles tiles, GsrTierLists tiers,
@@ -545,3 +557,9 @@
         });
     });
 }
+
+#pragma clang fp contract(off)
+#include "bwd_row_job.h"
+namespace {
+__device__ void bwd_row_job(const GsrRowJob& job, uint32_t w, int lane) { gsr::bwd_row_job_run(job, w, lane); }
+}
diff --git a/gaussiansplatting.jl_amd/csrc/gsr_api.cpp b/gaussiansplatting.jl_amd/csrc/gsr_api.cpp
--- a/gaussiansplatting.jl_amd/csrc/gsr_api.cpp
+++ b/gaussiansplatting.jl_amd/csrc/gsr_api.cpp
@@ -35,7 +35,7 @@
     }
 };
 
-constexpr int kHandleBufs = 33;
+constexpr int kHandleBufs = 34;
 
 bool valid_mode(int m) { return m == GSR_MODE_RGB || m == GSR_MODE_RGBD || m == GSR_MODE_RGBDN; }
 
@@ -57,6 +57,7 @@
     DevBuf bins, keys_compact, big_list, values_sorted, s0, s1, s2, s3, big_scratch, long_state;
     DevBuf overflow_fill;
     DevBuf rows, vmean2d;
+    DevBuf sh_jac;
     DevBuf pose_part;
     DevBuf d0, d1, d2, partial;
     uint32_t* host_totals = nullptr;
@@ -130,6 +131,7 @@
     BUF(dbg_flag, false, false, 1u),
     BUF(pose_part, true, true, 1u),
     BUF(comp, true, true, 1u),
+    BUF(sh_jac, true, true, 1u),
 };
 #undef BUF
 template <class Pred> constexpr int count_bufs(Pred pred) {
@@ -138,8 +140,8 @@
     return n;
 }
 static_assert(sizeof(kBufs) / sizeof(kBufs[0]) == kHandleBufs, "gsr_handle::all holds one pointer per row");
-static_assert(count_bufs([](const BufRow& r) { return r.scene; }) == 18, "the scene buffers");
-static_assert(count_bufs([](const BufRow& r) { return r.fill_ok; }) == 11, "the GSR_DEBUG_FILL candidates");
+static_assert(count_bufs([](const BufRow& r) { return r.scene; }) == 19, "the scene buffers");
+static_assert(count_bufs([](const BufRow& r) { return r.fill_ok; }) == 12, "the GSR_DEBUG_FILL candidates");
 static_assert(count_bufs([](const BufRow& r) { return r.guard_word == 0u; }) == 3, "the id buffers whose guard word is 0");
 
 bool antialiased(const gsr_handle* h) { return (h->cfg.flags & GSR_FLAG_ANTIALIASED) != 0u; }
@@ -702,7 +704,7 @@
 }
 
 static int launch_composite_bwd(gsr_handle* h, hipStream_t s, int C, const GsrCam& k, const float* background,
-                                const float* vpixels, bool color_only) {
+                                const float* vpixels, bool color_only, const GsrRowJob* job, bool* job_carried) {
     color_only = color_only && C > 3;
     gsr_bwd_split sp;
     gsr_policy_bwd_split(&h->pcfg, h->pol.tier_n[0], h->pol.tier_n[1], h->pol.tier_n[2], &sp);
@@ -720,7 +722,8 @@
                                         h->long_state.as<float>());
         HIPCHK(hipEventRecord(h->ev_join, h->aux_stream));
     }
-    gsr_launch_composite_bwd(s, C, k, tiles_of(h), stream_of(h), frame, vpixels, inst_of(h), tiers.split_len, color_only, accurate);
+    *job_carried = gsr_launch_composite_bwd(s, C, k, tiles_of(h), stream_of(h), frame, vpixels, inst_of(h), job, tiers.split_len,
+                                            color_only, accurate);
     if (n > 0) HIPCHK(hipStreamWaitEvent(s, h->ev_join, 0));
     return GSR_OK;
 }
@@ -740,15 +743,33 @@
 }
 
 static int composite_bwd_stage(gsr_handle* h, hipStream_t s, const gsr_inputs* in, const gsr_camera* cam, const float* vpixels,
-                               float* vmeans2d, uint32_t flags, GsrCam* k) {
+                               float* vmeans2d, uint32_t flags, GsrCam* k, const gsr_grads* grads, bool* job_carried) {
     int rc;
+    *job_carried = false;
     if (!vmeans2d && (rc = h->vmean2d.ensure(gaussian_bytes(h, in->n).vmean2d, 1.25f))) return rc;
     h->vmean2d_cur = vmeans2d ? reinterpret_cast<float2*>(vmeans2d) : h->vmean2d.as<float2>();
     const bool color_only = (flags & GSR_GRADS_COLOR_COTANGENT) != 0u;
     if (color_only && (rc = check_color_cotangent(h, vpixels, s))) return rc;
     *k = make_cam(h, cam);
+    GsrRowJob job{};
+    const bool bg_zero = in->background[0] == 0.0f && in->background[1] == 0.0f && in->background[2] == 0.0f;
+    if (grads && grads->vshs && !grads->vcolors && h->cfg.mode == 3 && bg_zero && h->cfg.grad_precision == GSR_DEFAULT &&
+        h->last_D > 0) {
+        gsr_bwd_row_job rj;
+        gsr_policy_bwd_row_job(&h->pcfg, in->n, &rj);
+        if ((rc = h->sh_jac.ensure(gaussian_bytes(h, in->n).sh_jac, 1.25f))) return rc;
+        job.n_wg = rj.n_wg; job.slice = rj.slice;
+        job.n = in->n; job.K = in->n_coeffs; job.degree = in->sh_degree;
+        job.means = in->means; job.shs = in->shs; job.radii = h->radii_cur;
+        for (int c = 0; c < 3; c++) job.center[c] = k->center[c];
+        job.jac = h->sh_jac.as<float>();
+        job.vmeans = grads->vmeans; job.vshs = grads->vshs; job.vopac = grads->vopacities; job.vscales = grads->vscales;
+        job.vrots = reinterpret_cast<float4*>(grads->vrotations);
+    }
     StageScope sc(h->prof, ST_COMPOSITE_BWD, s);
-    if (h->last_D > 0 && (rc = launch_composite_bwd(h, s, h->cfg.mode, *k, in->background, vpixels, color_only))) return rc;
+    if (h->last_D > 0 &&
+        (rc = launch_composite_bwd(h, s, h->cfg.mode, *k, in->background, vpixels, color_only, job.n_wg ? &job : nullptr, job_carried)))
+        return rc;
     sc.close();
     return GSR_OK;
 }
@@ -773,13 +794,14 @@
     if (n == 0) return GSR_OK;
     if (g->vR && (rc = h->pose_part.ensure(gaussian_bytes(h, n).pose_part, 1.25f))) return rc;
     GsrCam k;
-    if ((rc = composite_bwd_stage(h, s, in, cam, vpixels, g->vmeans2d, g->flags, &k))) return rc;
+    bool job_carried = false;
+    if ((rc = composite_bwd_stage(h, s, in, cam, vpixels, g->vmeans2d, g->flags, &k, g, &job_carried))) return rc;
     StageScope sc8(h->prof, ST_PERGAUSS_BWD, s);
     gsr_launch_pergauss_bwd(s, n, in->n_coeffs, in->sh_degree, C, in->means, in->scales, in->rotations, in->shs, k,
                             geom_of(h), inst_of(h), h->vmean2d_cur, g->vmeans, g->vshs, g->vopacities,
                             g->vscales, g->vrotations, g->vR, g->vt, h->pose_part.as<float>(), g->vcolors,
                             h->cfg.grad_precision == GSR_GRAD_FP32_REFERENCE,
-                            antialiased(h) ? in->opacities : nullptr, comp_of(h));
+                            antialiased(h) ? in->opacities : nullptr, comp_of(h), job_carried ? h->sh_jac.as<float>() : nullptr);
     sc8.close();
     HIPCHK(hipGetLastError());
     h->bwd_valid = true;
@@ -954,7 +976,8 @@
     hipStream_t s = (hipStream_t)stream_v;
     const int C = h->cfg.mode;
     GsrCam k;
-    if ((rc = composite_bwd_stage(h, s, in, cam, vpixels, st->vmeans2d, st->flags, &k))) return rc;
+    bool no_job = false;
+    if ((rc = composite_bwd_stage(h, s, in, cam, vpixels, st->vmeans2d, st->flags, &k, nullptr, &no_job))) return rc;
     StageScope sc12(h->prof, ST_PERGAUSS_BWD, s);
     const gsr::TailState S = gsr_make_tail_state(st->theta, st->mu, st->nu, lr_t, st->beta1, st->beta2, st->eps,
                                                  st->scale_dims, st->shs, st->opacities_act, st->scales_act);
diff --git a/gaussiansplatting.jl_amd/csrc/gsr_kernels.h b/gaussiansplatting.jl_amd/csrc/gsr_kernels.h
--- a/gaussiansplatting.jl_amd/csrc/gsr_kernels.h
+++ b/gaussiansplatting.jl_amd/csrc/gsr_kernels.h
@@ -91,7 +91,8 @@
                              float* pose_part ,
                              float* vcolors ,
                              bool fp32_chain ,
-                             const float* opac, const float* comp );
+                             const float* opac, const float* comp ,
+                             const float* sh_jac );
 namespace gsr { struct TailState; }
 void gsr_launch_pergauss_bwd_tail(hipStream_t s, int n, int K, int degree, int channels, GsrCam cam, GsrGeom geom,
                                   GsrInst inst, float2* vmean2d, const gsr::TailState& S, bool fp32_chain,
@@ -133,8 +134,17 @@
 void gsr_launch_sort_composite_fwd(hipStream_t s, int channels, GsrCam cam, GsrTiles tiles, GsrKeys keys, GsrGeom geom,
                                    GsrStream stream, GsrFrame frame, uint32_t cap_instances,
                                    bool keep_backward_state );
-void gsr_launch_composite_bwd(hipStream_t s, int channels, GsrCam cam, GsrTiles tiles, GsrStream stream, GsrFrame frame,
-                              const float* vpixels, GsrInst inst,
+struct GsrRowJob {
+    uint32_t first_wg;
+    uint32_t n_wg, slice;
+    int n, K, degree;
+    const float* means; const float* shs; const int32_t* radii;
+    float center[3];
+    float* jac;
+    float* vmeans; float* vshs; float* vopac; float* vscales; float4* vrots;
+};
+bool gsr_launch_composite_bwd(hipStream_t s, int channels, GsrCam cam, GsrTiles tiles, GsrStream stream, GsrFrame frame,
+                              const float* vpixels, GsrInst inst, const GsrRowJob* job ,
                               uint32_t split_len ,
                               bool color_only ,
                               bool accurate );
diff --git a/gaussiansplatting.jl_amd/csrc/gsr_policy.cpp b/gaussiansplatting.jl_amd/csrc/gsr_policy.cpp
--- a/gaussiansplatting.jl_amd/csrc/gsr_policy.cpp
+++ b/gaussiansplatting.jl_amd/csrc/gsr_policy.cpp
@@ -221,4 +221,15 @@
     if (n == 0) out->split_len = 0xFFFFFFFFu;
 }
 
-}
+void gsr_policy_bwd_row_job(const gsr_policy_config* cfg, int32_t n, gsr_bwd_row_job* out) {
+    (void)cfg;
+    out->n_wg = out->slice = 0;
+    if (n <= 0) return;
+    const uint32_t un = (uint32_t)n, target_wg = 512u;
+    uint32_t trips = (un + 64u * target_wg - 1u) / (64u * target_wg);
+    trips = trips < 4u ? 4u : trips > 32u ? 32u : trips;
+    out->slice = 64u * trips;
+    out->n_wg = (un + out->slice - 1u) / out->slice;
+}
+
+}
diff --git a/gaussiansplatting.jl_amd/csrc/gsr_sizes.h b/gaussiansplatting.jl_amd/csrc/gsr_sizes.h
--- a/gaussiansplatting.jl_amd/csrc/gsr_sizes.h
+++ b/gaussiansplatting.jl_amd/csrc/gsr_sizes.h
@@ -10,6 +10,7 @@
     size_t vmean2d;
     size_t pose_part;
     size_t comp;
+    size_t sh_jac;
 };
 
 inline gsr_gaussian_bytes gsr_sizes_per_gaussian(size_t n, int C, size_t pose_partial_floats, bool antialiased = false) {
@@ -22,6 +23,7 @@
     b.vmean2d = n * 8;
     b.pose_part = pose_partial_floats * 4;
     b.comp = antialiased ? nn * 4 : 0;
+    b.sh_jac = C == 3 ? n * 36 : 0;
     return b;
 }
 
diff --git a/gaussiansplatting.jl_amd/csrc/pergauss.hip b/gaussiansplatting.jl_amd/csrc/pergauss.hip
--- a/gaussiansplatting.jl_amd/csrc/pergauss.hip
+++ b/gaussiansplatting.jl_amd/csrc/pergauss.hip
@@ -366,13 +366,19 @@
     }
 }
 
-template <int DEG>
+template <int DEG, bool JAC = false>
 __device__ __forceinline__ void sh_bwd(const float* sh, const float p[3], const GsrCam& cam, const float vc[3], float b[16],
                                        float vmsh[3]) {
     float d0[3], dir[3];
     view_dir(p, cam.center, d0, dir);
     sh_basis<DEG>(dir, b);
     float dcx[3] = {0, 0, 0}, dcy[3] = {0, 0, 0}, dcz[3] = {0, 0, 0};
+    if constexpr (JAC) {
+        if (DEG > 0) {
+#pragma unroll
+            for (int c = 0; c < 3; c++) { dcx[c] = sh[c]; dcy[c] = sh[3 + c]; dcz[c] = sh[6 + c]; }
+        }
+    } else {
     if (DEG > 0) {
         const float x = dir[0], y = dir[1], z = dir[2];
 #pragma unroll
@@ -408,6 +414,7 @@
             }
         }
     }
+    }
     float vdir[3];
     vdir[0] = dcx[0] * vc[0] + dcx[1] * vc[1] + dcx[2] * vc[2];
     vdir[1] = dcy[0] * vc[0] + dcy[1] * vc[1] + dcy[2] * vc[2];
@@ -419,7 +426,7 @@
     vmsh[2] = (-d0[0] * d0[2] * vdir[0] - d0[1] * d0[2] * vdir[1] + (s2 - d0[2] * d0[2]) * vdir[2]) * inv_s;
 }
 
-template <bool FUSED>
+template <bool FUSED, bool JAC = false>
 __device__ __forceinline__ void store_or_apply_sh(int i, int n, int K, float* __restrict__ vshs, const float* vcolors,
                                                   const gsr::TailState& TS, const float f_b[16], const float f_vc[3],
                                                   int f_nb, const float f_vmean[3], float f_vopac, const float f_vs[3],
@@ -440,10 +447,12 @@
     if constexpr (!FUSED) {
         if (!vcolors) {
             __syncthreads();
-            store_sh_rows(vshs, i0, cnt, K3, [&](int il, int j) {
+            auto value = [&](int il, int j) {
                 const int k = j / 3, c = j - 3 * k;
                 return k < tail_nb[il] ? tail_b[il][k] * tail_vc[il][c] : 0.0f;
-            });
+            };
+            if constexpr (JAC) gsr::store_sh_rows_where(vshs, i0, cnt, K3, value, [&](int il) { return tail_nb[il] != 0; });
+            else store_sh_rows(vshs, i0, cnt, K3, value);
         }
     }
     if constexpr (FUSED) {
@@ -457,7 +466,7 @@
     }
 }
 
-template <int DEG, bool FUSED, bool F32CHAIN = false, bool AA = false>
+template <int DEG, bool FUSED, bool F32CHAIN = false, bool AA = false, bool JAC = false>
 __global__ __launch_bounds__(256, 1) void pergauss_bwd_kernel(int n, int K, int channels, const float* __restrict__ means,
                                                            const float* __restrict__ scales,
                                                            const float4* __restrict__ rots,
@@ -504,7 +513,7 @@
     if (i < n) {
         if (!visible) {
             vmean2d_out[i] = make_float2(0.0f, 0.0f);
-            if constexpr (!FUSED) {
+            if constexpr (!FUSED && !JAC) {
 #pragma unroll
                 for (int c = 0; c < 3; c++) { vmeans[3 * i + c] = 0.0f; vscales[3 * i + c] = 0.0f; }
                 vrots[i] = make_float4(0, 0, 0, 0);
@@ -555,12 +564,12 @@
                 for (int c = 0; c < 3; c++) vscales[3 * i + c] = vs[c];
             }
 
-            const float* sh = FUSED ? TS.rest + (size_t)3 * (K - 1) * i : shs + (size_t)3 * K * i + 3;
+            const float* sh = JAC ? shs + (size_t)9 * i : FUSED ? TS.rest + (size_t)3 * (K - 1) * i : shs + (size_t)3 * K * i + 3;
             const uint32_t clamp_bits = __float_as_uint(rec.q2.y);
             float vc[3] = {a0.x * (1.0f - (float)(clamp_bits & 1u)), a0.y * (1.0f - (float)((clamp_bits >> 1) & 1u)),
                            a0.z * (1.0f - (float)((clamp_bits >> 2) & 1u))};
             float b[16], vmsh[3];
-            sh_bwd<DEG>(sh, p, cam, vc, b, vmsh);
+            sh_bwd<DEG, JAC>(sh, p, cam, vc, b, vmsh);
             constexpr int NB = (DEG + 1) * (DEG + 1);
             if (!FUSED && vcolors) {
                 vcolors[3 * i] = vc[0]; vcolors[3 * i + 1] = vc[1]; vcolors[3 * i + 2] = vc[2];
@@ -577,7 +586,7 @@
             }
         }
     }
-    store_or_apply_sh<FUSED>(i, n, K, vshs, vcolors, TS, f_b, f_vc, f_nb, f_vmean, f_vopac, f_vs, f_vq);
+    store_or_apply_sh<FUSED, JAC>(i, n, K, vshs, vcolors, TS, f_b, f_vc, f_nb, f_vmean, f_vopac, f_vs, f_vq);
     if (pose_part) {
         __shared__ float pose_red[4][12];
 #pragma unroll
@@ -642,7 +651,7 @@
                              const float* scales, const float* rots, const float* shs, GsrCam cam, GsrGeom geom,
                              GsrInst inst, float2* vmean2d, float* vmeans, float* vshs, float* vopac,
                              float* vscales, float* vrots, float* vR, float* vt, float* pose_part, float* vcolors,
-                             bool fp32_chain, const float* opac, const float* comp) {
+                             bool fp32_chain, const float* opac, const float* comp, const float* sh_jac) {
     if (n <= 0) return;
     dim3 grid((n + 255) / 256), block(256);
     const float4* r4 = reinterpret_cast<const float4*>(rots);
@@ -654,6 +663,14 @@
             constexpr bool F32 = f;
             dispatch_bool(comp != nullptr, [&](auto a) {
                 constexpr bool AA = a;
+                if constexpr (!F32) {
+                    if (sh_jac && !vcolors) {
+                        hipLaunchKernelGGL((pergauss_bwd_kernel<DEG, false, false, AA, true>), grid, block, 0, s, n, K, channels, means,
+                                           scales, r4, sh_jac, cam, geom, inst, vmean2d, vmeans, vshs, vopac, vscales, vr4,
+                                           vR ? pose_part : nullptr, vcolors, none, opac, comp);
+                        return;
+                    }
+                }
                 hipLaunchKernelGGL((pergauss_bwd_kernel<DEG, false, F32, AA>), grid, block, 0, s, n, K, channels, means, scales,
                                    r4, shs, cam, geom, inst, vmean2d, vmeans, vshs, vopac, vscales, vr4,
                                    vR ? pose_part : nullptr, vcolors, none, opac, comp);
diff --git a/gaussiansplatting.jl_amd/csrc/sh_rows.h b/gaussiansplatting.jl_amd/csrc/sh_rows.h
--- a/gaussiansplatting.jl_amd/csrc/sh_rows.h
+++ b/gaussiansplatting.jl_amd/csrc/sh_rows.h
@@ -55,4 +55,22 @@
     for (int e = 4 * total4 + threadIdx.x; e < total; e += 256) dst[e] = element(e);
 }
 
+template <class Value, class Keep>
+__device__ __forceinline__ void store_sh_rows_where(float* __restrict__ vshs, int i0, int cnt, int K3, Value value, Keep keep) {
+    const uint32_t inv = (1u << 20) / (uint32_t)K3 + 1u;
+    float* __restrict__ dst = vshs + (size_t)i0 * K3;
+    const int total = cnt * K3;
+    auto owner = [&](int e) { return (int)(((uint32_t)e * inv) >> 20); };
+    auto element = [&](int e) {
+        const int il = owner(e);
+        return value(il, e - il * K3);
+    };
+    const int total4 = (((uintptr_t)dst & 15) == 0) ? total >> 2 : 0;
+    for (int f = threadIdx.x; f < total4; f += 256)
+        if (keep(owner(4 * f)) || keep(owner(4 * f + 3)))
+            reinterpret_cast<float4*>(dst)[f] = make_float4(element(4 * f), element(4 * f + 1), element(4 * f + 2), element(4 * f + 3));
+    for (int e = 4 * total4 + threadIdx.x; e < total; e += 256)
+        if (keep(owner(e))) dst[e] = element(e);
 }
+
+}
diff --git a/gaussiansplatting.jl_amd/csrc/splat_math.h b/gaussiansplatting.jl_amd/csrc/splat_math.h
--- a/gaussiansplatting.jl_amd/csrc/splat_math.h
+++ b/gaussiansplatting.jl_amd/csrc/splat_math.h
@@ -146,4 +146,46 @@
     dir[0] = d0[0] * inv; dir[1] = d0[1] * inv; dir[2] = d0[2] * inv;
 }
 
+template <int DEG>
+__device__ __forceinline__ void sh_dir_jacobian(const float* sh, const float dir[3], float dcx[3], float dcy[3], float dcz[3]) {
+    auto coeff = [&](int k, int c) { return sh[3 * (k - 1) + c]; };
+#pragma unroll
+    for (int c = 0; c < 3; c++) { dcx[c] = 0.0f; dcy[c] = 0.0f; dcz[c] = 0.0f; }
+    if (DEG > 0) {
+        const float x = dir[0], y = dir[1], z = dir[2];
+#pragma unroll
+        for (int c = 0; c < 3; c++) {
+            dcx[c] = -SH1 * coeff(3, c); dcy[c] = -SH1 * coeff(1, c); dcz[c] = SH1 * coeff(2, c);
+        }
+        if (DEG > 1) {
+            float x2 = x * x, y2 = y * y, z2 = z * z, xy = x * y, xz = x * z, yz = y * z;
+#pragma unroll
+            for (int c = 0; c < 3; c++) {
+                dcx[c] = dcx[c] + SH2C1 * y * coeff(4, c) + SH2C3 * 2.0f * -x * coeff(6, c) +
+                         SH2C4 * z * coeff(7, c) + SH2C5 * 2.0f * x * coeff(8, c);
+                dcy[c] = dcy[c] + SH2C1 * x * coeff(4, c) + SH2C2 * z * coeff(5, c) +
+                         SH2C3 * 2.0f * -y * coeff(6, c) + SH2C5 * 2.0f * -y * coeff(8, c);
+                dcz[c] = dcz[c] + SH2C2 * y * coeff(5, c) + SH2C3 * 4.0f * z * coeff(6, c) +
+                         SH2C4 * x * coeff(7, c);
+            }
+            if (DEG > 2) {
+#pragma unroll
+                for (int c = 0; c < 3; c++) {
+                    dcx[c] = dcx[c] + SH3C1 * coeff(9, c) * 3.0f * 2.0f * xy + SH3C2 * coeff(10, c) * yz +
+                             SH3C3 * coeff(11, c) * -2.0f * xy + SH3C4 * coeff(12, c) * -3.0f * 2.0f * xz +
+                             SH3C5 * coeff(13, c) * (-3.0f * x2 + 4.0f * z2 - y2) +
+                             SH3C6 * coeff(14, c) * 2.0f * xz + SH3C7 * coeff(15, c) * 3.0f * (x2 - y2);
+                    dcy[c] = dcy[c] + SH3C1 * coeff(9, c) * 3.0f * (x2 - y2) + SH3C2 * coeff(10, c) * xz +
+                             SH3C3 * coeff(11, c) * (-3.0f * y2 + 4.0f * z2 - x2) +
+                             SH3C4 * coeff(12, c) * -3.0f * 2.0f * yz + SH3C5 * coeff(13, c) * -2.0f * xy +
+                             SH3C6 * coeff(14, c) * -2.0f * yz + SH3C7 * coeff(15, c) * -3.0f * 2.0f * xy;
+                    dcz[c] = dcz[c] + SH3C2 * coeff(10, c) * xy + SH3C3 * coeff(11, c) * 4.0f * 2.0f * yz +
+                             SH3C4 * coeff(12, c) * 3.0f * (2.0f * z2 - x2 - y2) +
+                             SH3C5 * coeff(13, c) * 4.0f * 2.0f * xz + SH3C6 * coeff(14, c) * (x2 - y2);
+                }
+            }
+        }
+    }
 }
+
+}
diff --git a/include/gsr_policy.h b/include/gsr_policy.h
--- a/include/gsr_policy.h
+++ b/include/gsr_policy.h
@@ -113,6 +113,11 @@
 GSR_API void gsr_policy_bwd_split(const gsr_policy_config* cfg, uint32_t n_mid4, uint32_t n_mid8, uint32_t n_big,
                                   gsr_bwd_split* out);
 
+typedef struct gsr_bwd_row_job {
+    uint32_t n_wg, slice;
+} gsr_bwd_row_job;
+GSR_API void gsr_policy_bwd_row_job(const gsr_policy_config* cfg, int32_t n, gsr_bwd_row_job* out);
+
 #ifdef __cplusplus
 }
 #endif
```

After: 1623, median of 6. 1.2% higher.
